# MariMamgo/CNN-with-PDE

Measured on AMD Instinct MI355X. Metric: PDE-layer fwd+bwd Msamples/s, higher is better.
Workload: dtype f32; 1 GPU; cifar10.EnhancedDiffusionLayer(size=32, channels=64, num_steps=10) fwd+bwd, 30 implicit sweeps, batch 512/GPU, channel mixing disabled (BASELINE configs[1], SURVEY §8d cfg2 primary); global_batch=512, parallelism=dp1, grad_allreduce_bytes=0, rccl_world_size=1

## Files before the change

cnn-with-pde_amd/csrc/blob_to_inc.py:

```python
#!/usr/bin/env python3
import sys

if "--fwd" in sys.argv:
    sys.argv.remove("--fwd")
    with open(sys.argv[1], "w") as out:
        rows = []
        for spec in sys.argv[2:]:
            name, path = spec.split("=", 1)
            data = open(path, "rb").read()
            out.write(f"alignas(4096) static const unsigned char kAsmFwdBlob_{name}[{len(data)}] = {{\n")
            for i in range(0, len(data), 32):
                out.write(",".join(str(b) for b in data[i:i + 32]) + ",\n")
            out.write("};\n")
            rows.append(f'    {{"{name}", {int(name.rstrip("t"))}, kAsmFwdBlob_{name}, "adi_fwd_asm_n32_w{name}", {{}}, {{}}}},')
        out.write("static Variant g_fwd_variants[] = {\n" + "\n".join(rows) + "\n};\n")
    sys.exit(0)

with open(sys.argv[1], "w") as out:
    rows = []
    for spec in sys.argv[2:]:
        name, path = spec.split("=", 1)
        data = open(path, "rb").read()
        nw = int(name.split("a")[0].rstrip("b"))
        out.write(f"alignas(4096) static const unsigned char kAsmBlob_{name}[{len(data)}] = {{\n")
        for i in range(0, len(data), 32):
            out.write(",".join(str(b) for b in data[i:i + 32]) + ",\n")
        out.write("};\n")
        rows.append(f'    {{"{name}", {nw}, kAsmBlob_{name}, "adi_bwd_asm_n32_w{name}", {{}}, {{}}}},')
    out.write("static Variant g_variants[] = {\n" + "\n".join(rows) + "\n};\n")
```

cnn-with-pde_amd/csrc/gen_adi_bwd_asm.py:

```python
#!/usr/bin/env python3
import sys

N = 32
M = 16
LINE = 36
IMG_B = 32 * LINE * 4
REC_STRIDE = 5 * 32 * LINE + 32
BWD_OFF_B = (32 * LINE) * 4
REC_WIN = 3 * 32 * LINE + 32
PIECES = (REC_WIN * 4 + 1023) // 1024
RECP_B = PIECES * 1024
OFF_JN = 0
OFF_E = 32 * 4
OFF_INV = (32 * LINE + 32) * 4
OFF_KAP = (2 * 32 * LINE + 32) * 4
NSLOT = 6
RING_B = NSLOT * RECP_B
TAB_DTS = 96 * 4
TAB_FIRST = 2 * 96 * 4
PLANE_B = N * N * 4


class Emit:
    def __init__(self):
        self.out = []
        self.lgkm = []
        self.vm = []
        self.smem = False
        self.nvalu = 0
        self.vop2_only = False

    def raw(self, s, comment=None):
        self.out.append("\t" + s + (f"\t; {comment}" if comment else ""))

    def label(self, name):
        self.out.append(f"{name}:")

    def comment(self, s):
        self.out.append(f"\t; {s}")

    @staticmethod
    def _last_hit(queue, regs):
        for i in range(len(queue) - 1, -1, -1):
            if queue[i] & regs:
                return i
        return None

    def need(self, regs):
        regs = set(regs)
        i = self._last_hit(self.lgkm, regs)
        if i is not None:
            n = len(self.lgkm) - 1 - i
            if self.smem:
                n = 0
            n = min(n, 15)
            self.raw(f"s_waitcnt lgkmcnt({n})")
            self.lgkm = self.lgkm[len(self.lgkm) - n:] if n else []
            if n == 0:
                self.smem = False
        i = self._last_hit(self.vm, regs)
        if i is not None:
            n = min(len(self.vm) - 1 - i, 63)
            self.raw(f"s_waitcnt vmcnt({n})")
            self.vm = self.vm[len(self.vm) - n:] if n else []

    def drain(self, vm=True, lgkm=True):
        parts = []
        if vm:
            parts.append("vmcnt(0)")
            self.vm = []
        if lgkm:
            parts.append("lgkmcnt(0)")
            self.lgkm = []
            self.smem = False
        self.raw("s_waitcnt " + " ".join(parts))

    def assert_idle(self):
        assert not self.lgkm and not self.vm and not self.smem, (len(self.lgkm), len(self.vm), self.smem)

    def valu(self, text, dst=(), src=(), comment=None):
        if self.vop2_only and text.startswith("v_fma_f32 "):
            ops = [o.strip() for o in text[len("v_fma_f32 "):].split(",")]
            text = f"v_fmac_f32 {ops[0]}, {ops[1].lstrip('-')}, {ops[2]}"
        self.need(set(dst) | set(src))
        self.raw(text, comment)
        self.nvalu += 1

    def salu(self, text, comment=None):
        self.raw(text, comment)

    def ds_read(self, text, dst, addr):
        self.need(set(dst) | {addr})
        self.raw(text)
        self.lgkm.append(set(dst))

    def ds_write(self, text, data, addr):
        self.need(set(data) | {addr})
        self.raw(text)
        self.lgkm.append(set())

    def vm_load(self, text, dst, addr):
        self.need(set(dst) | {addr})
        self.raw(text)
        self.vm.append(set(dst))

    def vm_store(self, text, data, addr):
        self.need(set(data) | {addr})
        self.raw(text)
        self.vm.append(set())

    def s_load(self, text):
        self.raw(text)
        self.smem = True
        self.lgkm.append(set())


def v(n):
    return f"v{n}"


def vq(n):
    return f"v[{n}:{n + 3}]"


def vp(n):
    return f"v[{n}:{n + 1}]"


def gen(NW, ABL=0, MODE="A"):
    """MODE "A": <= 168 VGPRs (three waves per SIMD with 12-wave workgroups), coefficient rows streamed four values at a time,
    one re-layout image per wave.  MODE "B": 256 VGPRs (two waves per SIMD, 8-wave workgroups): the three coefficient rows of
    a sweep are HELD in registers — fetched for the NEXT sweep as the current sweep's pass frees them, kept across the twin x
    sweeps of neighbouring time steps —, two images per wave so that the re-layout writes ride inside the G passes, the next
    chunk's planes prefetched into 64 registers during the chunk's last time step, the time-weighted sums updated in the
    latency shadow of the next sweep's junction exchange."""
    assert NW in (8, 12, 16) and MODE in ("A", "B")
    BM = MODE == "B"
    NT = NW * 64
    PPI = 2 * NW
    NPI = (3 * PIECES + NW - 1) // NW
    NIMG = 2 if BM else 1
    WIMG_B = NIMG * IMG_B
    IMG0 = 0
    RING0 = NW * WIMG_B
    ADT = BM and bool(ABL & 65536)
    assert (NW - 1) * WIMG_B < 65536
    FLAGS = BM and not (ABL & 16384)
    CNT0 = RING0 + RING_B
    LDS_TOTAL = CNT0 + (16 if FLAGS else 0)
    assert LDS_TOTAL <= 163840, LDS_TOTAL
    assert (NW - 1) * WIMG_B < 65536
    e = Emit()
    e.vop2_only = bool(ABL & 64)
    name = f"adi_bwd_asm_n32_w{NW}" + ("b" if BM else "") + (f"a{ABL}" if ABL else "")

    NMARK = 16

    def mark(i):
        if not (ABL & 4096):
            return
        assert i < NMARK
        lab = f"L_mark_{mark.n}"
        mark.n += 1
        e.drain(vm=False)
        e.salu(f"s_or_b32 s{S_T0}, s2, s3")
        e.salu(f"s_or_b32 s{S_T0}, s{S_T0}, s4")
        e.salu(f"s_sub_u32 s{S_T1}, s{S_Q}, s{S_G}")
        e.salu(f"s_xor_b32 s{S_T1}, s{S_T1}, s{S_g}")
        e.salu(f"s_or_b32 s{S_T0}, s{S_T0}, s{S_T1}")
        e.salu(f"s_xor_b32 s{S_T1}, s{S_KK}, 5")
        e.salu(f"s_or_b32 s{S_T0}, s{S_T0}, s{S_T1}")
        e.salu(f"s_cmp_lg_u32 s{S_T0}, 0")
        e.salu(f"s_cbranch_scc1 {lab}")
        e.raw(f"{'s_memrealtime' if ABL & 131072 else 's_memtime'} s[{S_STAMP}:{S_STAMP + 1}]")
        e.raw("s_waitcnt lgkmcnt(0)")
        a, b = NQ[0][0], NQ[0][1]
        e.raw(f"v_mov_b32 {v(a)}, s{S_STAMP}")
        e.raw(f"v_mov_b32 {v(b)}, s{S_STAMP + 1}")
        e.salu(f"s_mul_i32 s{S_T1}, s{S_WAVE}, {NMARK * 8}")
        e.salu(f"s_add_u32 s{S_T1}, s{S_T1}, {i * 8}")
        e.raw(f"v_mov_b32 {v(VADDR)}, s{S_T1}")
        assert NQ[0][1] == NQ[0][0] + 1 and NQ[0][0] % 2 == 0
        e.raw(f"global_store_dwordx2 {v(VADDR)}, v[{a}:{b}], s[{S_DBG}:{S_DBG + 1}]")
        e.raw("s_waitcnt vmcnt(0)")
        e.label(lab)
    mark.n = 0

    def stage(n):
        e.salu(f"s_cmp_eq_u32 s31, {n}")
        e.salu("s_cbranch_scc1 L_end")

    nv = [0]

    def alloc(n, align=1):
        nv[0] = (nv[0] + align - 1) // align * align
        r = nv[0]
        nv[0] += n
        return r

    R = [alloc(16, 4), alloc(16, 4)]
    X = [alloc(16, 4), alloc(16, 4)]
    AX, TX, AY, TY = alloc(16, 4), alloc(16, 4), alloc(16, 4), alloc(16, 4)
    if BM:
        CE, CI, CK = alloc(16, 4), alloc(16, 4), alloc(16, 4)
        EB = [CE, CE + 4]
        IB = [CI, CI + 4]
        KB = [CK, CK + 4]
    else:
        EB = [alloc(4, 4), alloc(4, 4)]
        IB = [alloc(4, 4), alloc(4, 4)]
        KB = [alloc(4, 4), alloc(4, 4)]
    _nq = alloc(4, 2)
    NQ = [[_nq, _nq + 1], [_nq + 2, _nq + 3]]
    JN = alloc(1)
    VADDR = alloc(1)
    if BM:
        VADDRN = alloc(1)
        VDTS = alloc(1)
    V_CROW = alloc(1)
    V_TWR = alloc(1)
    V_TRD = alloc(1)
    V_NKK, V_MU, V_MD = alloc(1), alloc(1), alloc(1)
    V_LANE16 = alloc(1)
    V_M2 = alloc(1)
    if BM:
        PF = alloc(64, 4)
        TQ = [CE + 4 * i for i in range(4)] + [CI + 4 * i for i in range(4)] + [CK + 4 * i for i in range(4)]
    else:
        TQ = [EB[0], EB[1], IB[0], IB[1], KB[0], KB[1]]
    NVGPR = nv[0]
    assert NVGPR <= (256 if BM else 168), NVGPR

    S_GY, S_Y, S_GU, S_COEF, S_PART, S_TAB, S_VAR = 8, 10, 12, 14, 16, 18, 20
    S_B, S_C, S_S, S_G, S_GUSC, S_ACCP, S_CZ, S_K, S_NCHUNK = 22, 23, 24, 25, 26, 27, 28, 29, 30
    S_c, S_g, S_WAVE, S_T, S_Q, S_KK, S_SET, S_MORE = 32, 33, 34, 35, 36, 37, 38, 39
    S_T0, S_T1, S_T2, S_T3 = 40, 41, 42, 43
    S_FIRSTX, S_FIRSTY, S_TLX, S_TLY = 44, 45, 46, 47
    S_SRC, S_SRC0 = 48, 50
    S_KKN = 52
    S_SWB, S_SWB3 = 53, 54
    S_DL = [56 + 2 * i for i in range(6)]
    S_DS = [57 + 2 * i for i in range(6)]
    S_PV = 68
    S_HASNEXT = 69
    S_PX = 55
    S_TSTEP = 5
    S_PB = [70, 72, 74, 76]
    S_VAL0, S_VAL1 = 78, 79
    S_DTS = [80, 81, 82]
    S_DTSB = 84
    S_REC = 86
    S_SS = 87
    S_A0 = 88
    S_IT = 90
    S_DBG = 92
    S_STAMP = 94
    NSGPR = 96

    e.out.append('\t.amdgcn_target "amdgcn-amd-amdhsa--gfx950"')
    e.out.append("\t.amdhsa_code_object_version 6")
    e.out.append("\t.text")
    e.out.append(f"\t.protected\t{name}")
    e.out.append(f"\t.globl\t{name}")
    e.out.append("\t.p2align\t8")
    e.out.append(f"\t.type\t{name},@function")
    e.label(name)

    e.s_load("s_load_dwordx16 s[8:23], s[0:1], 0x0")
    e.s_load("s_load_dwordx8 s[24:31], s[0:1], 0x40")
    if ABL & 4096:
        e.s_load(f"s_load_dwordx2 s[{S_DBG}:{S_DBG + 1}], s[0:1], 0x60")
    T0, T1, T2 = EB[0], EB[0] + 1, EB[0] + 2
    e.valu(f"v_bfe_u32 {v(T1)}, v0, 6, 4", dst=[T1])
    e.valu(f"v_and_b32 {v(T0)}, 63, v0", dst=[T0])
    e.raw("s_nop 1")
    e.valu(f"v_readfirstlane_b32 s{S_WAVE}, {v(T1)}", src=[T1])
    e.valu(f"v_lshlrev_b32 {v(V_LANE16)}, 4, {v(T0)}", dst=[V_LANE16], src=[T0])
    e.valu(f"v_and_b32 {v(T1)}, 31, {v(T0)}", dst=[T1], src=[T0])
    e.valu(f"v_lshrrev_b32 {v(T2)}, 5, {v(T0)}", dst=[T2], src=[T0])
    e.valu(f"v_mul_u32_u24 {v(V_CROW)}, 0x90, {v(T1)}", dst=[V_CROW], src=[T1])
    e.valu(f"v_lshl_add_u32 {v(V_CROW)}, {v(T2)}, 6, {v(V_CROW)}", dst=[V_CROW], src=[T2, V_CROW])
    T3 = EB[0] + 3
    e.valu(f"v_sub_u32 {v(T3)}, 47, {v(T1)}", dst=[T3], src=[T1])
    e.valu(f"v_cmp_gt_u32 vcc, 16, {v(T1)}", src=[T1])
    e.valu(f"v_cndmask_b32 {v(T3)}, {v(T3)}, {v(T1)}, vcc", dst=[T3], src=[T3, T1])
    e.salu(f"s_mul_i32 s{S_T}, s{S_WAVE}, {WIMG_B}")
    e.salu(f"s_add_u32 s{S_T}, s{S_T}, {IMG0}")
    e.valu(f"v_mul_u32_u24 {v(V_TWR)}, 0x900, {v(T2)}", dst=[V_TWR], src=[T2])
    e.valu(f"v_lshl_add_u32 {v(V_TWR)}, {v(T3)}, 2, {v(V_TWR)}", dst=[V_TWR], src=[T3, V_TWR])
    e.valu(f"v_add_u32 {v(V_TWR)}, s{S_T}, {v(V_TWR)}", dst=[V_TWR], src=[V_TWR])
    if ADT:
        TA, TB = IB[0], IB[0] + 1
        e.valu(f"v_sub_u32 {v(TA)}, 31, {v(T1)}", dst=[TA], src=[T1])
        e.valu(f"v_cmp_gt_u32 vcc, 16, {v(T1)}", src=[T1])
        e.valu(f"v_cndmask_b32 {v(TA)}, {v(TA)}, {v(T1)}, vcc", dst=[TA], src=[TA, T1])
        e.valu(f"v_cndmask_b32 {v(TB)}, 1, 0, vcc", dst=[TB])
        e.valu(f"v_add_u32 {v(V_TRD)}, 4, {v(TA)}", dst=[V_TRD], src=[TA])
        e.valu(f"v_lshrrev_b32 {v(V_TRD)}, 3, {v(V_TRD)}", dst=[V_TRD], src=[V_TRD])
        e.valu(f"v_lshl_add_u32 {v(V_TRD)}, {v(V_TRD)}, 3, {v(TA)}", dst=[V_TRD], src=[V_TRD, TA])
        e.valu(f"v_lshlrev_b32 {v(TA)}, 6, {v(TA)}", dst=[TA], src=[TA])
        e.valu(f"v_lshl_add_u32 {v(V_TRD)}, {v(V_TRD)}, 2, {v(TA)}", dst=[V_TRD], src=[V_TRD, TA])
        e.valu(f"v_lshl_add_u32 {v(V_TRD)}, {v(TB)}, 5, {v(V_TRD)}", dst=[V_TRD], src=[TB, V_TRD])
        e.valu(f"v_lshl_add_u32 {v(V_TRD)}, {v(T2)}, 4, {v(V_TRD)}", dst=[V_TRD], src=[T2, V_TRD])
        e.valu(f"v_lshlrev_b32 {v(V_TRD)}, 2, {v(V_TRD)}", dst=[V_TRD], src=[V_TRD])
        e.valu(f"v_add_u32 {v(V_TRD)}, s{S_T}, {v(V_TRD)}", dst=[V_TRD], src=[V_TRD])
    else:
        e.valu(f"v_mul_u32_u24 {v(V_TRD)}, 0x90, {v(T3)}", dst=[V_TRD], src=[T3])
        e.valu(f"v_lshl_add_u32 {v(V_TRD)}, {v(T2)}, 6, {v(V_TRD)}", dst=[V_TRD], src=[T2, V_TRD])
        e.valu(f"v_add_u32 {v(V_TRD)}, s{S_T}, {v(V_TRD)}", dst=[V_TRD], src=[V_TRD])
    e.valu(f"v_cmp_lt_u32 vcc, 0, {v(T1)}", src=[T1])
    e.valu(f"v_cndmask_b32 {v(V_MU)}, 0, 1.0, vcc", dst=[V_MU])
    e.valu(f"v_cmp_gt_u32 vcc, 31, {v(T1)}", src=[T1])
    e.valu(f"v_cndmask_b32 {v(V_MD)}, 0, 1.0, vcc", dst=[V_MD])
    e.valu(f"v_add_f32 {v(V_NKK)}, {v(V_MU)}, {v(V_MD)}", dst=[V_NKK], src=[V_MU, V_MD])
    e.valu(f"v_sub_f32 {v(V_NKK)}, 0, {v(V_NKK)}", dst=[V_NKK], src=[V_NKK])
    e.valu(f"v_mov_b32 {v(V_M2)}, -2.0", dst=[V_M2])
    for k in range(16):
        for a in (AX, TX, AY, TY):
            e.valu(f"v_mov_b32 {v(a + k)}, 0", dst=[a + k])
    for i in range(4):
        e.valu(f"v_mov_b32 {v(IB[0] + i)}, 0", dst=[IB[0] + i])
    e.valu(f"v_add_u32 {v(VADDR)}, s{S_T}, {v(V_LANE16)}", dst=[VADDR], src=[V_LANE16])
    for i in range(4):
        e.ds_write(f"ds_write_b128 {v(VADDR)}, {vq(IB[0])} offset:{1024 * i}", [IB[0] + j for j in range(4)], VADDR)
    e.valu(f"v_lshrrev_b32 {v(T0)}, 1, {v(V_LANE16)}", dst=[T0], src=[V_LANE16])
    e.valu(f"v_add_u32 {v(T0)}, s{S_T}, {v(T0)}", dst=[T0], src=[T0])
    e.ds_write(f"ds_write_b64 {v(T0)}, {vp(IB[0])} offset:4096", [IB[0], IB[0] + 1], T0)
    if BM:
        for i in range(4):
            e.ds_write(f"ds_write_b128 {v(VADDR)}, {vq(IB[0])} offset:{IMG_B + 1024 * i}", [IB[0] + j for j in range(4)], VADDR)
        e.ds_write(f"ds_write_b64 {v(T0)}, {vp(IB[0])} offset:{IMG_B + 4096}", [IB[0], IB[0] + 1], T0)
    e.drain(vm=False)
    stage(1)
    e.salu(f"s_mul_i32 s{S_T0}, s{S_CZ}, s4")
    e.salu(f"s_add_u32 s{S_c}, s2, s{S_T0}")
    e.salu(f"s_mov_b32 s{S_g}, s3")
    e.salu(f"s_lshl_b32 s{S_T0}, s{S_c}, 2")
    e.salu(f"s_add_u32 s{S_A0}, s{S_VAR}, s{S_T0}")
    e.salu(f"s_addc_u32 s{S_A0 + 1}, s{S_VAR + 1}, 0")
    e.s_load(f"s_load_dword s{S_T1}, s[{S_A0}:{S_A0 + 1}], 0x0")
    e.s_load(f"s_load_dwordx4 s[{S_FIRSTX}:{S_FIRSTX + 3}], s[{S_TAB}:{S_TAB + 1}], {hex(TAB_FIRST)}")
    e.drain(vm=False)
    e.salu(f"s_cmp_lg_u32 s{S_T1}, 0")
    e.salu("s_cbranch_scc1 L_end")
    stage(2)
    e.salu(f"s_add_u32 s{S_DTSB}, s{S_TAB}, {TAB_DTS}")
    e.salu(f"s_addc_u32 s{S_DTSB + 1}, s{S_TAB + 1}, 0")
    e.salu(f"s_mul_i32 s{S_SWB}, s{S_C}, {REC_STRIDE * 4}")
    e.salu(f"s_mul_i32 s{S_SWB3}, s{S_SWB}, 3")
    e.salu(f"s_mul_i32 s{S_T0}, s{S_c}, {REC_STRIDE * 4}")
    e.salu(f"s_mul_hi_u32 s{S_T1}, s{S_c}, {REC_STRIDE * 4}")
    e.salu(f"s_add_u32 s{S_T0}, s{S_T0}, {BWD_OFF_B}")
    e.salu(f"s_addc_u32 s{S_T1}, s{S_T1}, 0")
    e.salu(f"s_add_u32 s{S_SRC0}, s{S_COEF}, s{S_T0}")
    e.salu(f"s_addc_u32 s{S_SRC0 + 1}, s{S_COEF + 1}, s{S_T1}")
    e.salu(f"s_mov_b32 s{S_PV}, 0")
    e.salu(f"s_mov_b32 s{S_PX}, 0")
    for i in range(NPI):
        e.salu(f"s_add_u32 s{S_T0}, s{S_WAVE}, {NW * i}")
        e.salu(f"s_mul_i32 s{S_T1}, s{S_T0}, 4682")
        e.salu(f"s_lshr_b32 s{S_T1}, s{S_T1}, 16")
        e.salu(f"s_mul_i32 s{S_T2}, s{S_T1}, {PIECES}")
        e.salu(f"s_sub_u32 s{S_T2}, s{S_T0}, s{S_T2}")
        e.salu(f"s_lshl_b32 s{S_T2}, s{S_T2}, 10")
        e.salu(f"s_mul_i32 s{S_T3}, s{S_T1}, {RECP_B}")
        e.salu(f"s_add_u32 s{S_DL[i]}, s{S_T3}, s{S_T2}")
        e.salu(f"s_add_u32 s{S_DL[i]}, s{S_DL[i]}, {RING0}")
        e.salu(f"s_sub_u32 s{S_T3}, 2, s{S_T1}")
        e.salu(f"s_mul_i32 s{S_T3}, s{S_T3}, s{S_SWB}")
        e.salu(f"s_add_u32 s{S_DS[i]}, s{S_T3}, s{S_T2}")
        e.salu(f"s_cmp_lt_u32 s{S_T0}, {3 * PIECES}")
        e.salu(f"s_cselect_b32 s{S_T3}, {1 << i}, 0")
        e.salu(f"s_or_b32 s{S_PV}, s{S_PV}, s{S_T3}")
        e.salu(f"s_cmp_eq_u32 s{S_T1}, 0")
        e.salu(f"s_cselect_b32 s{S_T3}, {1 << i}, 0")
        e.salu(f"s_or_b32 s{S_PX}, s{S_PX}, s{S_T3}")

    def dma_step(kk_sgpr, set_expr_sgpr, skip_twin=False):
        e.salu(f"s_mul_i32 s{S_T0}, s{kk_sgpr}, s{S_SWB3}")
        e.salu(f"s_add_u32 s{S_SRC}, s{S_SRC0}, s{S_T0}")
        e.salu(f"s_addc_u32 s{S_SRC + 1}, s{S_SRC0 + 1}, 0")
        if skip_twin:
            e.salu(f"s_sub_u32 s{S_T0}, s{S_K}, 1")
            e.salu(f"s_cmp_eq_u32 s{kk_sgpr}, s{S_T0}")
            e.salu(f"s_cselect_b32 s{S_T1}, 0, s{S_PX}")
            e.salu(f"s_bitcmp1_b32 s{S_ACCP}, 1")
            e.salu(f"s_cselect_b32 s{S_T1}, s{S_T1}, 0")
            e.salu(f"s_andn2_b32 s{S_T3}, s{S_PV}, s{S_T1}")
        for i in range(NPI):
            last_partial = (NW * i + NW > 3 * PIECES)
            if skip_twin:
                e.salu(f"s_bitcmp1_b32 s{S_T3}, {i}")
                e.salu(f"s_cbranch_scc0 L_nodma_{dma_step.n}_{i}")
            elif last_partial:
                e.salu(f"s_bitcmp1_b32 s{S_PV}, {i}")
                e.salu(f"s_cbranch_scc0 L_nodma_{dma_step.n}_{i}")
            e.salu(f"s_add_u32 s{S_A0}, s{S_SRC}, s{S_DS[i]}")
            e.salu(f"s_addc_u32 s{S_A0 + 1}, s{S_SRC + 1}, 0")
            e.salu(f"s_add_u32 m0, s{set_expr_sgpr}, s{S_DL[i]}")
            e.salu("s_nop 0")
            e.raw(f"global_load_lds_dwordx4 {v(V_LANE16)}, s[{S_A0}:{S_A0 + 1}]")
            if last_partial or skip_twin:
                e.label(f"L_nodma_{dma_step.n}_{i}")
        dma_step.n += 1
    dma_step.n = 0

    def load_dts(kk_sgpr):
        e.salu(f"s_mul_i32 s{S_T0}, s{kk_sgpr}, 12")
        e.salu(f"s_add_u32 s{S_A0}, s{S_DTSB}, s{S_T0}")
        e.salu(f"s_addc_u32 s{S_A0 + 1}, s{S_DTSB + 1}, 0")
        e.s_load(f"s_load_dword s{S_DTS[0]}, s[{S_A0}:{S_A0 + 1}], 0x0")
        e.s_load(f"s_load_dword s{S_DTS[1]}, s[{S_A0}:{S_A0 + 1}], 0x4")
        e.s_load(f"s_load_dword s{S_DTS[2]}, s[{S_A0}:{S_A0 + 1}], 0x8")

    def flag_add(which, set_sgpr_is_other):
        a = VDTS
        e.salu(f"s_cmp_eq_u32 s{S_SET}, 0")
        e.salu(f"s_cselect_b32 s{S_T0}, {4 if set_sgpr_is_other else 0}, {0 if set_sgpr_is_other else 4}")
        e.salu(f"s_add_u32 s{S_T0}, s{S_T0}, {CNT0 + which * 8}")
        e.valu(f"v_mov_b32 {v(a)}, s{S_T0}", dst=[a])
        b = VADDR
        e.valu(f"v_mov_b32 {v(b)}, 1", dst=[b])
        e.need({a, b})
        e.raw("s_mov_b64 exec, 1")
        e.raw(f"ds_add_u32 {v(a)}, {v(b)}")
        e.raw("s_mov_b64 exec, -1")
        e.lgkm.append(set())

    def flag_wait(which, other_set, target_sgpr, tag):
        a, b = VDTS, VADDR
        e.drain(vm=False)
        e.salu(f"s_cmp_eq_u32 s{S_SET}, 0")
        e.salu(f"s_cselect_b32 s{S_T0}, {4 if other_set else 0}, {0 if other_set else 4}")
        e.salu(f"s_add_u32 s{S_T0}, s{S_T0}, {CNT0 + which * 8}")
        e.valu(f"v_mov_b32 {v(a)}, s{S_T0}", dst=[a])
        e.salu(f"s_mov_b32 s{S_T1}, 0")
        e.label(f"L_poll_{tag}")
        e.raw(f"ds_read_b32 {v(b)}, {v(a)}")
        e.raw("s_waitcnt lgkmcnt(0)")
        e.raw(f"v_readfirstlane_b32 s{S_T2}, {v(b)}")
        e.salu(f"s_cmp_ge_u32 s{S_T2}, s{target_sgpr}")
        e.salu(f"s_cbranch_scc1 L_polled_{tag}")
        e.salu(f"s_add_u32 s{S_T1}, s{S_T1}, 1")
        e.salu(f"s_cmp_lt_u32 s{S_T1}, 0x100000")
        e.salu(f"s_cbranch_scc0 L_polled_{tag}")
        e.raw("s_sleep 1")
        e.salu(f"s_branch L_poll_{tag}")
        e.label(f"L_polled_{tag}")

    if FLAGS:
        for i in range(4):
            e.valu(f"v_mov_b32 {v(IB[0] + i)}, 0", dst=[IB[0] + i])
        e.valu(f"v_mov_b32 {v(VADDR)}, {CNT0}", dst=[VADDR])
        e.ds_write(f"ds_write_b128 {v(VADDR)}, {vq(IB[0])}", [IB[0] + j for j in range(4)], VADDR)
        e.salu(f"s_mov_b32 s{S_TSTEP}, 0")
    if bool(ABL & 8192) != BM:
        e.salu(f"s_cmp_lt_u32 s{S_WAVE}, {NW // 2}")
        e.salu("s_cbranch_scc1 L_noprio")
        e.raw("s_setprio 1")
        e.label("L_noprio")
    stage(31)
    e.salu(f"s_mov_b32 s{S_SET}, 0")
    e.salu(f"s_sub_u32 s{S_KK}, s{S_K}, 1")
    dma_step(S_KK, S_SET)
    e.raw("s_waitcnt vmcnt(0)")
    stage(32)
    load_dts(S_KK)
    e.drain(vm=False)
    stage(33)
    e.salu(f"s_mov_b32 s{S_Q}, s{S_g}")
    e.drain()
    e.raw("s_barrier")
    if FLAGS:
        flag_add(0, False)
    stage(3)

    def plane_bases(ptr, dst_pairs, q_sgpr=None):
        q_sgpr = S_Q if q_sgpr is None else q_sgpr
        for j, d in enumerate(dst_pairs):
            e.salu(f"s_mul_i32 s{S_T0}, s{q_sgpr}, {PPI}")
            e.salu(f"s_lshl_b32 s{S_T1}, s{S_WAVE}, 1")
            e.salu(f"s_add_u32 s{S_T0}, s{S_T0}, s{S_T1}")
            if j:
                e.salu(f"s_add_u32 s{S_T0}, s{S_T0}, {j}")
            e.salu(f"s_sub_u32 s{S_T1}, s{S_B}, 1")
            e.salu(f"s_min_u32 s{S_T0}, s{S_T0}, s{S_T1}")
            e.salu(f"s_mul_i32 s{S_T0}, s{S_T0}, s{S_C}")
            e.salu(f"s_add_u32 s{S_T0}, s{S_T0}, s{S_c}")
            e.salu(f"s_lshr_b32 s{S_T1}, s{S_T0}, 20")
            e.salu(f"s_lshl_b32 s{S_T0}, s{S_T0}, 12")
            e.salu(f"s_add_u32 s{d}, s{ptr}, s{S_T0}")
            e.salu(f"s_addc_u32 s{d + 1}, s{ptr + 1}, s{S_T1}")

    def io_addresses():
        a, b = NQ[0][0], NQ[0][1]
        e.salu("s_mov_b32 vcc_lo, 0xf0f0f0f0")
        e.salu("s_mov_b32 vcc_hi, 0xf0f0f0f0")
        e.valu(f"v_lshrrev_b32 {v(a)}, 7, {v(V_LANE16)}", dst=[a], src=[V_LANE16])
        e.valu(f"v_mul_u32_u24 {v(a)}, 0x90, {v(a)}", dst=[a], src=[a])
        e.valu(f"v_and_b32 {v(b)}, 0x70, {v(V_LANE16)}", dst=[b], src=[V_LANE16])
        e.valu(f"v_sub_u32 {v(VADDR)}, 0xb0, {v(b)}", dst=[VADDR], src=[b])
        e.valu(f"v_cndmask_b32 {v(b)}, {v(b)}, {v(VADDR)}, vcc", dst=[b], src=[b, VADDR])
        e.valu(f"v_add3_u32 {v(VADDR)}, {v(a)}, {v(b)}, s{S_T}", dst=[VADDR], src=[a, b])
        e.valu(f"v_add_u32 {v(JN)}, s{S_T}, {v(V_CROW)}", dst=[JN], src=[V_CROW])

    def chunk_flags():
        e.salu(f"s_add_u32 s{S_T0}, s{S_Q}, s{S_G}")
        e.salu(f"s_cmp_lt_u32 s{S_T0}, s{S_NCHUNK}")
        e.salu(f"s_cselect_b32 s{S_MORE}, 1, 0")
        e.salu(f"s_mul_i32 s{S_T0}, s{S_Q}, {PPI}")
        e.salu(f"s_lshl_b32 s{S_T1}, s{S_WAVE}, 1")
        e.salu(f"s_add_u32 s{S_T0}, s{S_T0}, s{S_T1}")
        e.salu(f"s_cmp_lt_u32 s{S_T0}, s{S_B}")
        e.salu(f"s_cselect_b32 s{S_VAL0}, 1, 0")
        e.salu(f"s_add_u32 s{S_T0}, s{S_T0}, 1")
        e.salu(f"s_cmp_lt_u32 s{S_T0}, s{S_B}")
        e.salu(f"s_cselect_b32 s{S_VAL1}, 1, 0")

    def fetch_planes(regs, q_sgpr, tracked):
        plane_bases(S_GY, [S_PB[0], S_PB[1]], q_sgpr)
        plane_bases(S_Y, [S_PB[2], S_PB[3]], q_sgpr)
        for d, pb in zip(regs, S_PB):
            for i in range(4):
                text = f"global_load_dwordx4 {vq(d + 4 * i)}, {v(V_LANE16)}, s[{pb}:{pb + 1}] offset:{1024 * i} nt"
                if tracked:
                    e.vm_load(text, [d + 4 * i + j for j in range(4)], V_LANE16)
                else:
                    e.raw(text)

    def place_planes(regs):
        dests = [R[0], R[1], X[0], X[1]]
        io_addresses()
        for pi, (src, d) in enumerate(zip(regs, dests)):
            for i in range(4):
                t = TQ[(pi * 4 + i) % len(TQ)]
                a = src + 4 * i
                e.valu(f"v_cndmask_b32 {v(t)}, {v(a)}, {v(a + 3)}, vcc", dst=[t], src=[a, a + 3])
                e.valu(f"v_cndmask_b32 {v(t + 1)}, {v(a + 1)}, {v(a + 2)}, vcc", dst=[t + 1], src=[a + 1, a + 2])
                e.valu(f"v_cndmask_b32 {v(t + 2)}, {v(a + 2)}, {v(a + 1)}, vcc", dst=[t + 2], src=[a + 2, a + 1])
                e.valu(f"v_cndmask_b32 {v(t + 3)}, {v(a + 3)}, {v(a)}, vcc", dst=[t + 3], src=[a + 3, a])
                e.ds_write(f"ds_write_b128 {v(VADDR)}, {vq(t)} offset:{8 * LINE * 4 * i}", [t + j for j in range(4)], VADDR)
            for i in range(4):
                e.ds_read(f"ds_read_b128 {vq(d + 4 * i)}, {v(JN)} offset:{16 * i}", [d + 4 * i + j for j in range(4)], JN)
        e.drain(vm=False)
        for pj, sval in ((0, S_VAL0), (1, S_VAL1)):
            e.salu(f"s_cmp_eq_u32 s{sval}, 1")
            e.salu(f"s_cbranch_scc1 L_valid_{place_planes.n}_{pj}")
            for k in range(16):
                e.valu(f"v_mov_b32 {v(R[pj] + k)}, 0", dst=[R[pj] + k])
                e.valu(f"v_mov_b32 {v(X[pj] + k)}, 0", dst=[X[pj] + k])
            e.label(f"L_valid_{place_planes.n}_{pj}")
        place_planes.n += 1
    place_planes.n = 0

    def load_planes():
        e.comment("---- chunk in: gy -> R, y -> X (global -> natural image -> half rows)")
        chunk_flags()
        if BM:
            place_planes([PF, PF + 16, PF + 32, PF + 48])
        else:
            regs = [R[0], R[1], X[0], X[1]]
            fetch_planes(regs, S_Q, True)
            place_planes(regs)

    def store_planes():
        e.comment("---- chunk out: gu = R * (1+eps)^-S (half rows -> natural image -> global)")
        e.assert_idle()
        plane_bases(S_GU, [S_PB[0], S_PB[1]])
        io_addresses()
        for pj, sval in ((0, S_VAL0), (1, S_VAL1)):
            e.salu(f"s_cmp_eq_u32 s{sval}, 0")
            e.salu(f"s_cbranch_scc1 L_nostore_{store_planes.n}_{pj}")
            for k in range(16):
                e.valu(f"v_mul_f32 {v(R[pj] + k)}, s{S_GUSC}, {v(R[pj] + k)}", dst=[R[pj] + k], src=[R[pj] + k])
            for i in range(4):
                e.ds_write(f"ds_write_b128 {v(JN)}, {vq(R[pj] + 4 * i)} offset:{16 * i}", [R[pj] + 4 * i + j for j in range(4)], JN)
            for i in range(4):
                e.ds_read(f"ds_read_b128 {vq(X[pj] + 4 * i)}, {v(VADDR)} offset:{8 * LINE * 4 * i}",
                          [X[pj] + 4 * i + j for j in range(4)], VADDR)
            for i in range(4):
                a = X[pj] + 4 * i
                t = R[pj] + 4 * i
                e.valu(f"v_cndmask_b32 {v(t)}, {v(a)}, {v(a + 3)}, vcc", dst=[t], src=[a, a + 3])
                e.valu(f"v_cndmask_b32 {v(t + 1)}, {v(a + 1)}, {v(a + 2)}, vcc", dst=[t + 1], src=[a + 1, a + 2])
                e.valu(f"v_cndmask_b32 {v(t + 2)}, {v(a + 2)}, {v(a + 1)}, vcc", dst=[t + 2], src=[a + 2, a + 1])
                e.valu(f"v_cndmask_b32 {v(t + 3)}, {v(a + 3)}, {v(a)}, vcc", dst=[t + 3], src=[a + 3, a])
                e.raw(f"global_store_dwordx4 {v(V_LANE16)}, {vq(t)}, s[{S_PB[pj]}:{S_PB[pj] + 1}] offset:{1024 * i} nt")
            e.drain(vm=False)
            e.label(f"L_nostore_{store_planes.n}_{pj}")
        store_planes.n += 1
    store_planes.n = 0

    def q4(k):
        return k // 4

    def ebuf(k):
        return EB[q4(k) & 1] + (k & 3)

    def ibuf(k):
        return IB[q4(k) & 1] + (k & 3)

    def kbuf(k):
        return KB[q4(k) & 1] + (k & 3)

    def rd_quad(buf, off, q):
        if ABL & 2:
            return
        b = buf[q & 1]
        e.ds_read(f"ds_read_b128 {vq(b)}, {v(VADDR)} offset:{off + 16 * q}", [b + j for j in range(4)], VADDR)

    def sweep_addr(rec_index):
        e.salu(f"s_add_u32 s{S_REC}, s{S_SET}, {rec_index * RECP_B + RING0}")
        e.valu(f"v_add_u32 {v(VADDR)}, s{S_REC}, {v(V_CROW)}", dst=[VADDR], src=[V_CROW])
        t = NQ[0][0]
        e.valu(f"v_bfe_u32 {v(t)}, {v(V_LANE16)}, 2, 7", dst=[t], src=[V_LANE16])
        e.valu(f"v_add_u32 {v(t)}, s{S_REC}, {v(t)}", dst=[t], src=[t])
        if not (ABL & 2):
            e.ds_read(f"ds_read_b32 {v(JN)}, {v(t)} offset:{OFF_JN}", [JN], t)

    def xchg_pair(a, b):
        e.need({a, b})
        if ABL & 128:
            return
        if not (ABL & 32):
            e.raw("s_nop 1")
        e.raw(f"v_permlane32_swap_b32 {v(a)}, {v(b)}")
        if not (ABL & 32):
            e.raw("s_nop 1")
        e.raw(f"v_permlane32_swap_b32 {v(b)}, {v(a)}")
        if not (ABL & 32):
            e.raw("s_nop 1")
        e.nvalu += 2

    def h_pass(issue_hooks):
        for k in range(1, 16):
            for p in (0, 1):
                e.valu(f"v_fmac_f32 {v(R[p] + k)}, {v(ebuf(k - 1))}, {v(R[p] + k - 1)}",
                       dst=[R[p] + k], src=[R[p] + k, ebuf(k - 1), R[p] + k - 1])
            if k in issue_hooks:
                issue_hooks[k]()

    def junction():
        ta, tb = NQ[0][0], NQ[1][0]
        e.valu(f"v_mul_f32 {v(ta)}, {v(ebuf(15))}, {v(R[0] + 15)}", dst=[ta], src=[ebuf(15), R[0] + 15])
        e.valu(f"v_mul_f32 {v(tb)}, {v(ebuf(15))}, {v(R[1] + 15)}", dst=[tb], src=[ebuf(15), R[1] + 15])
        xchg_pair(ta, tb)
        e.valu(f"v_add_f32 {v(R[0] + 15)}, {v(R[0] + 15)}, {v(tb)}", dst=[R[0] + 15], src=[R[0] + 15, tb])
        e.valu(f"v_add_f32 {v(R[1] + 15)}, {v(R[1] + 15)}, {v(ta)}", dst=[R[1] + 15], src=[R[1] + 15, ta])
        e.valu(f"v_mul_f32 {v(R[0] + 15)}, {v(JN)}, {v(R[0] + 15)}", dst=[R[0] + 15], src=[JN, R[0] + 15])
        e.valu(f"v_mul_f32 {v(R[1] + 15)}, {v(JN)}, {v(R[1] + 15)}", dst=[R[1] + 15], src=[JN, R[1] + 15])

    def t_update(acc, tacc, dts_sgpr, first_sgpr, tlast_sgpr, tag):
        if ABL & 256:
            return
        lab = f"L_tu_{tag}_{t_update.n}"
        t_update.n += 1
        e.salu(f"s_cmp_eq_u32 s{S_SS}, s{first_sgpr}")
        e.salu(f"s_cselect_b32 s{S_T0}, s{S_MORE}, 0")
        e.salu(f"s_and_b32 s{S_T1}, s{dts_sgpr}, 0x7fffffff")
        e.salu(f"s_or_b32 s{S_T1}, s{S_T1}, s{S_T0}")
        e.salu(f"s_cmp_eq_u32 s{S_T1}, 0")
        e.salu(f"s_cbranch_scc1 {lab}_skip")
        e.valu(f"v_mov_b32 {v(JN)}, s{dts_sgpr}", dst=[JN])
        e.salu(f"s_cmp_eq_u32 s{S_T0}, 0")
        e.salu(f"s_cbranch_scc1 {lab}_noadj")
        e.valu(f"v_subrev_f32 {v(JN)}, s{tlast_sgpr}, {v(JN)}", dst=[JN], src=[JN])
        e.label(f"{lab}_noadj")
        for k in range(16):
            e.valu(f"v_fmac_f32 {v(tacc + k)}, {v(JN)}, {v(acc + k)}", dst=[tacc + k], src=[tacc + k, JN, acc + k])
        e.label(f"{lab}_skip")
    t_update.n = 0

    def sweep_x(rec_index, dts_sgpr):
        e.comment(f"==== x sweep, record {rec_index} of the set")
        sweep_addr(rec_index)
        rd_quad(EB, OFF_E, 0)
        rd_quad(EB, OFF_E, 1)
        rd_quad(IB, OFF_INV, 3)
        rd_quad(KB, OFF_KAP, 3)
        rd_quad(IB, OFF_INV, 2)
        rd_quad(KB, OFF_KAP, 2)
        e.valu(f"v_mov_b32 {v(NQ[0][1])}, {v(X[0] + 15)}", dst=[NQ[0][1]], src=[X[0] + 15])
        e.valu(f"v_mov_b32 {v(NQ[1][1])}, {v(X[1] + 15)}", dst=[NQ[1][1]], src=[X[1] + 15])
        xchg_pair(NQ[0][1], NQ[1][1])
        XIN = [NQ[1][1], NQ[0][1]]
        h_pass({4: lambda: rd_quad(EB, OFF_E, 2), 8: lambda: rd_quad(EB, OFF_E, 3)})
        junction()
        def nqreg(p, k):
            if k == 15:
                return XIN[p]
            return NQ[p][k & 1]
        pend = None
        for k in range(15, -1, -1):
            for p in (0, 1):
                nq = nqreg(p, k)
                if k == 15:
                    e.valu(f"v_add_f32 {v(nq)}, {v(nq)}, {v(X[p] + 14)}", dst=[nq], src=[nq, X[p] + 14])
                    e.valu(f"v_fmac_f32 {v(nq)}, {v(V_M2)}, {v(X[p] + 15)}", dst=[nq], src=[nq, V_M2, X[p] + 15])
                elif k == 0:
                    e.valu(f"v_sub_f32 {v(nq)}, {v(X[p] + 1)}, {v(X[p])}", dst=[nq], src=[X[p] + 1, X[p]])
                else:
                    e.valu(f"v_add_f32 {v(nq)}, {v(X[p] + k - 1)}, {v(X[p] + k + 1)}", dst=[nq], src=[X[p] + k - 1, X[p] + k + 1])
                    e.valu(f"v_fmac_f32 {v(nq)}, {v(V_M2)}, {v(X[p] + k)}", dst=[nq], src=[nq, V_M2, X[p] + k])
            if pend is not None:
                kk = pend
                for p in (0, 1):
                    e.valu(f"v_fma_f32 {v(X[p] + kk)}, -{v(kbuf(kk))}, {v(nqreg(p, kk))}, {v(X[p] + kk)}",
                           dst=[X[p] + kk], src=[kbuf(kk), nqreg(p, kk), X[p] + kk])
                if kk in (12, 8):
                    rd_quad(KB, OFF_KAP, q4(kk) - 2)
            if k >= 1:
                for p in (0, 1):
                    e.valu(f"v_fmac_f32 {v(R[p] + k - 1)}, {v(ebuf(k))}, {v(R[p] + k)}",
                           dst=[R[p] + k - 1], src=[R[p] + k - 1, ebuf(k), R[p] + k])
                if k in (12, 8):
                    rd_quad(EB, OFF_E, q4(k) - 2)
            for p in (0, 1):
                e.valu(f"v_mul_f32 {v(R[p] + k)}, {v(ibuf(k))}, {v(R[p] + k)}", dst=[R[p] + k], src=[ibuf(k), R[p] + k])
            if k in (12, 8):
                rd_quad(IB, OFF_INV, q4(k) - 2)
            for p in (0, 1):
                e.valu(f"v_fmac_f32 {v(AX + k)}, {v(R[p] + k)}, {v(nqreg(p, k))}", dst=[AX + k], src=[AX + k, R[p] + k, nqreg(p, k)])
            pend = k
        for p in (0, 1):
            e.valu(f"v_fma_f32 {v(X[p])}, -{v(kbuf(0))}, {v(nqreg(p, 0))}, {v(X[p])}", dst=[X[p]], src=[kbuf(0), nqreg(p, 0), X[p]])
        t_update(AX, TX, dts_sgpr, S_FIRSTX, S_TLX, "x")

    def relayout(arr):
        if ABL & 1:
            return
        for p in (0, 1):
            for k in range(16):
                e.ds_write(f"ds_write_b32 {v(V_TWR)}, {v(arr[p] + k)} offset:{k * LINE * 4}", [arr[p] + k], V_TWR)
            for i in range(4):
                e.ds_read(f"ds_read_b128 {vq(arr[p] + 4 * i)}, {v(V_TRD)} offset:{16 * i}", [arr[p] + 4 * i + j for j in range(4)], V_TRD)

    def sweep_y(rec_index, dts_sgpr):
        e.comment(f"==== y sweep, record {rec_index} of the set")
        sweep_addr(rec_index)
        rd_quad(EB, OFF_E, 0)
        rd_quad(EB, OFF_E, 1)
        rd_quad(IB, OFF_INV, 3)
        rd_quad(IB, OFF_INV, 2)
        relayout(R)
        h_pass({4: lambda: rd_quad(EB, OFF_E, 2), 8: lambda: rd_quad(EB, OFF_E, 3)})
        junction()
        for k in range(15, -1, -1):
            if k >= 1:
                for p in (0, 1):
                    e.valu(f"v_fmac_f32 {v(R[p] + k - 1)}, {v(ebuf(k))}, {v(R[p] + k)}",
                           dst=[R[p] + k - 1], src=[R[p] + k - 1, ebuf(k), R[p] + k])
                if k in (12, 8):
                    rd_quad(EB, OFF_E, q4(k) - 2)
            for p in (0, 1):
                e.valu(f"v_mul_f32 {v(R[p] + k)}, {v(ibuf(k))}, {v(R[p] + k)}", dst=[R[p] + k], src=[ibuf(k), R[p] + k])
            if k in (12, 8):
                rd_quad(IB, OFF_INV, q4(k) - 2)
        rd_quad(KB, OFF_KAP, 0)
        rd_quad(KB, OFF_KAP, 1)
        relayout(R)
        order = [(k, p) for k in range(16) for p in (0, 1)]
        GRP = 4
        for g0 in range(0, len(order), GRP):
            grp = order[g0:g0 + GRP]
            regs = [NQ[0][0], NQ[0][1], NQ[1][0], NQ[1][1]]
            for (k, p), nq in zip(grp, regs):
                e.valu(f"v_mul_f32 {v(nq)}, {v(V_NKK)}, {v(X[p] + k)}", dst=[nq], src=[V_NKK, X[p] + k])
            dpp_u = "" if ABL & 16 else " wave_shr:1 row_mask:0xf bank_mask:0xf bound_ctrl:0"
            dpp_d = "" if ABL & 16 else " wave_shl:1 row_mask:0xf bank_mask:0xf bound_ctrl:0"
            opc = "v_fmac_f32" if ABL & 16 else "v_fmac_f32_dpp"
            for (k, p), nq in zip(grp, regs):
                e.valu(f"{opc} {v(nq)}, {v(X[p] + k)}, {v(V_MU)}{dpp_u}", dst=[nq], src=[nq, X[p] + k, V_MU])
            for (k, p), nq in zip(grp, regs):
                e.valu(f"{opc} {v(nq)}, {v(X[p] + k)}, {v(V_MD)}{dpp_d}", dst=[nq], src=[nq, X[p] + k, V_MD])
            for (k, p), nq in zip(grp, regs):
                e.valu(f"v_fmac_f32 {v(AY + k)}, {v(R[p] + k)}, {v(nq)}", dst=[AY + k], src=[AY + k, R[p] + k, nq])
            for (k, p), nq in zip(grp, regs):
                e.valu(f"v_fma_f32 {v(X[p] + k)}, -{v(kbuf(k))}, {v(nq)}, {v(X[p] + k)}", dst=[X[p] + k], src=[kbuf(k), nq, X[p] + k])
            klast = grp[-1][0]
            if klast in (3, 7) and grp[-1][1] == 1:
                rd_quad(KB, OFF_KAP, q4(klast) + 2)
        t_update(AY, TY, dts_sgpr, S_FIRSTY, S_TLY, "y")

    def rd_row(base, off, q, addr):
        if ABL & 2:
            return
        e.ds_read(f"ds_read_b128 {vq(base + 4 * q)}, {v(addr)} offset:{off + 16 * q}", [base + 4 * q + j for j in range(4)], addr)

    def rec_addr(vreg, rec_index):
        e.salu(f"s_add_u32 s{S_REC}, s{S_SET}, {rec_index * RECP_B + RING0}")
        e.valu(f"v_add_u32 {v(vreg)}, s{S_REC}, {v(V_CROW)}", dst=[vreg], src=[V_CROW])

    def rd_jn(rec_index):
        if ABL & 2:
            return
        e.salu(f"s_add_u32 s{S_T0}, s{S_SET}, {rec_index * RECP_B + RING0}")
        e.valu(f"v_bfe_u32 {v(VDTS)}, {v(V_LANE16)}, 2, 7", dst=[VDTS], src=[V_LANE16])
        e.valu(f"v_add_u32 {v(VDTS)}, s{S_T0}, {v(VDTS)}", dst=[VDTS], src=[VDTS])
        e.ds_read(f"ds_read_b32 {v(JN)}, {v(VDTS)} offset:{OFF_JN}", [JN], VDTS)

    def load_rows_now(rec_index):
        rec_addr(VADDR, rec_index)
        rd_jn(rec_index)
        for q in range(4):
            rd_row(CE, OFF_E, q, VADDR)
        for q in range(4):
            rd_row(CI, OFF_INV, q, VADDR)
        for q in range(4):
            rd_row(CK, OFF_KAP, q, VADDR)

    def t_update_b(acc, tacc, dts_sgpr, first_sgpr, tlast_sgpr, ss_delta, tag):
        if ABL & 256:
            return
        lab = f"L_tub_{tag}_{t_update_b.n}"
        t_update_b.n += 1
        e.salu(f"s_add_u32 s{S_T2}, s{S_SS}, {ss_delta}")
        e.salu(f"s_cmp_eq_u32 s{S_T2}, s{first_sgpr}")
        e.salu(f"s_cselect_b32 s{S_T0}, s{S_MORE}, 0")
        e.salu(f"s_and_b32 s{S_T1}, s{dts_sgpr}, 0x7fffffff")
        e.salu(f"s_or_b32 s{S_T1}, s{S_T1}, s{S_T0}")
        e.salu(f"s_cmp_eq_u32 s{S_T1}, 0")
        e.salu(f"s_cbranch_scc1 {lab}_skip")
        e.valu(f"v_mov_b32 {v(VDTS)}, s{dts_sgpr}", dst=[VDTS])
        e.salu(f"s_cmp_eq_u32 s{S_T0}, 0")
        e.salu(f"s_cbranch_scc1 {lab}_noadj")
        e.valu(f"v_subrev_f32 {v(VDTS)}, s{tlast_sgpr}, {v(VDTS)}", dst=[VDTS], src=[VDTS])
        e.label(f"{lab}_noadj")
        for k in range(16):
            e.valu(f"v_fmac_f32 {v(tacc + k)}, {v(VDTS)}, {v(acc + k)}", dst=[tacc + k], src=[tacc + k, VDTS, acc + k])
        e.label(f"{lab}_skip")
    t_update_b.n = 0

    def swap(a, b):
        if ABL & 128:
            return
        e.need({a, b})
        e.raw(f"v_permlane32_swap_b32 {v(a)}, {v(b)}")
        e.nvalu += 1

    def nop2():
        if not (ABL & 32):
            e.raw("s_nop 1")

    def h_link(k):
        for p in (0, 1):
            e.valu(f"v_fmac_f32 {v(R[p] + k)}, {v(CE + k - 1)}, {v(R[p] + k - 1)}", dst=[R[p] + k], src=[R[p] + k, CE + k - 1, R[p] + k - 1])

    def junction_b(shadow1=None, shadow2=None, shadow3=None):
        ta, tb = NQ[0][0], NQ[1][0]
        e.valu(f"v_mul_f32 {v(ta)}, {v(CE + 15)}, {v(R[0] + 15)}", dst=[ta], src=[CE + 15, R[0] + 15])
        e.valu(f"v_mul_f32 {v(tb)}, {v(CE + 15)}, {v(R[1] + 15)}", dst=[tb], src=[CE + 15, R[1] + 15])
        if shadow1:
            shadow1()
        nop2()
        swap(ta, tb)
        if shadow2:
            shadow2()
        else:
            nop2()
        swap(tb, ta)
        if shadow3:
            shadow3()
        else:
            nop2()
        e.valu(f"v_add_f32 {v(R[0] + 15)}, {v(R[0] + 15)}, {v(tb)}", dst=[R[0] + 15], src=[R[0] + 15, tb])
        e.valu(f"v_add_f32 {v(R[1] + 15)}, {v(R[1] + 15)}, {v(ta)}", dst=[R[1] + 15], src=[R[1] + 15, ta])
        e.valu(f"v_mul_f32 {v(R[0] + 15)}, {v(JN)}, {v(R[0] + 15)}", dst=[R[0] + 15], src=[JN, R[0] + 15])
        e.valu(f"v_mul_f32 {v(R[1] + 15)}, {v(JN)}, {v(R[1] + 15)}", dst=[R[1] + 15], src=[JN, R[1] + 15])

    W2 = bool(ABL & 32768)

    ADT_P = [0, 1, 2, 3, 12, 13, 14, 15, 16, 17, 18, 19, 28, 29, 30, 31]

    def relayout_bases(upper):
        if ADT and not (ABL & 1):
            if upper:
                e.salu(f"s_mov_b32 m0, s{S_T}")
            return
        if not W2 or (ABL & 1):
            return
        if upper:
            e.valu(f"v_add_u32 {v(VDTS)}, {8 * LINE * 4}, {v(V_TWR)}", dst=[VDTS], src=[V_TWR])
            e.valu(f"v_add_u32 {v(VADDR)}, {8 * LINE * 4 + IMG_B}, {v(V_TWR)}", dst=[VADDR], src=[V_TWR])
        else:
            e.valu(f"v_add_u32 {v(VADDR)}, {IMG_B}, {v(V_TWR)}", dst=[VADDR], src=[V_TWR])

    def relayout_write(p, k):
        if ABL & 1:
            return
        if ADT:
            e.need({R[p] + k})
            e.raw(f"ds_write_addtid_b32 {v(R[p] + k)} offset:{4 * (64 * k + 4 * ADT_P[k]) + p * IMG_B}")
            e.lgkm.append(set())
            return
        if not W2:
            e.ds_write(f"ds_write_b32 {v(V_TWR)}, {v(R[p] + k)} offset:{k * LINE * 4 + p * IMG_B}", [R[p] + k], V_TWR)
            return
        if k & 1:
            return
        if k >= 8:
            base = VDTS if p == 0 else VADDR
        else:
            base = V_TWR if p == 0 else VADDR
        o0 = (k % 8) * LINE
        e.ds_write(f"ds_write2_b32 {v(base)}, {v(R[p] + k)}, {v(R[p] + k + 1)} offset0:{o0} offset1:{o0 + LINE}",
                   [R[p] + k, R[p] + k + 1], base)

    def relayout_reads():
        if ABL & 1:
            return
        for p in (0, 1):
            for i in range(4):
                e.ds_read(f"ds_read_b128 {vq(R[p] + 4 * i)}, {v(V_TRD)} offset:{16 * i + p * IMG_B}",
                          [R[p] + 4 * i + j for j in range(4)], V_TRD)

    def relayout_fix():
        if not ADT or (ABL & 1):
            return
        e.need(set(range(R[0], R[0] + 16)) | set(range(R[1], R[1] + 16)))
        e.raw("s_mov_b32 exec_lo, 0")
        for p in (0, 1):
            for j in range(8):
                e.raw(f"v_swap_b32 {v(R[p] + j)}, {v(R[p] + 15 - j)}")
                e.nvalu += 1
        e.raw("s_mov_b32 exec_lo, -1")

    def sweep_x_b(rec_index, next_rec, relayout_after, deferred, own_t):
        e.comment(f"==== x sweep (held rows), record {rec_index} of the set")
        if next_rec is not None:
            rec_addr(VADDRN, next_rec)
        e.valu(f"v_mov_b32 {v(NQ[0][1])}, {v(X[0] + 15)}", dst=[NQ[0][1]], src=[X[0] + 15])
        e.valu(f"v_mov_b32 {v(NQ[1][1])}, {v(X[1] + 15)}", dst=[NQ[1][1]], src=[X[1] + 15])
        h_link(1)
        swap(NQ[0][1], NQ[1][1])
        h_link(2)
        swap(NQ[1][1], NQ[0][1])
        XIN = [NQ[1][1], NQ[0][1]]
        for k in range(3, 16):
            h_link(k)

        def nqreg(p, k):
            return XIN[p] if k == 15 else NQ[p][k & 1]

        def nq15_a():
            for p in (0, 1):
                nq = nqreg(p, 15)
                e.valu(f"v_add_f32 {v(nq)}, {v(nq)}, {v(X[p] + 14)}", dst=[nq], src=[nq, X[p] + 14])

        def nq15_b():
            for p in (0, 1):
                nq = nqreg(p, 15)
                e.valu(f"v_fmac_f32 {v(nq)}, {v(V_M2)}, {v(X[p] + 15)}", dst=[nq], src=[nq, V_M2, X[p] + 15])

        sh1 = (lambda: t_update_b(*deferred)) if deferred else None
        junction_b(sh1, nq15_a, nq15_b)
        if next_rec is not None:
            rd_jn(next_rec)
        if relayout_after:
            relayout_bases(True)
        pend = None
        for k in range(15, -1, -1):
            if relayout_after and k == 7:
                relayout_bases(False)
            if k < 15:
                for p in (0, 1):
                    nq = nqreg(p, k)
                    if k == 0:
                        e.valu(f"v_sub_f32 {v(nq)}, {v(X[p] + 1)}, {v(X[p])}", dst=[nq], src=[X[p] + 1, X[p]])
                    else:
                        e.valu(f"v_add_f32 {v(nq)}, {v(X[p] + k - 1)}, {v(X[p] + k + 1)}", dst=[nq], src=[X[p] + k - 1, X[p] + k + 1])
                        e.valu(f"v_fmac_f32 {v(nq)}, {v(V_M2)}, {v(X[p] + k)}", dst=[nq], src=[nq, V_M2, X[p] + k])
            if pend is not None:
                kk_ = pend
                for p in (0, 1):
                    e.valu(f"v_fma_f32 {v(X[p] + kk_)}, -{v(CK + kk_)}, {v(nqreg(p, kk_))}, {v(X[p] + kk_)}",
                           dst=[X[p] + kk_], src=[CK + kk_, nqreg(p, kk_), X[p] + kk_])
                if next_rec is not None and kk_ % 4 == 0:
                    rd_row(CK, OFF_KAP, kk_ // 4, VADDRN)
            if k >= 1:
                for p in (0, 1):
                    e.valu(f"v_fmac_f32 {v(R[p] + k - 1)}, {v(CE + k)}, {v(R[p] + k)}", dst=[R[p] + k - 1], src=[R[p] + k - 1, CE + k, R[p] + k])
                if next_rec is not None:
                    if k % 4 == 0:
                        rd_row(CE, OFF_E, k // 4, VADDRN)
                    elif k == 1:
                        rd_row(CE, OFF_E, 0, VADDRN)
            for p in (0, 1):
                e.valu(f"v_mul_f32 {v(R[p] + k)}, {v(CI + k)}, {v(R[p] + k)}", dst=[R[p] + k], src=[CI + k, R[p] + k])
            if next_rec is not None and k % 4 == 0:
                rd_row(CI, OFF_INV, k // 4, VADDRN)
            if relayout_after:
                for p in (0, 1):
                    relayout_write(p, k)
            for p in (0, 1):
                e.valu(f"v_fmac_f32 {v(AX + k)}, {v(R[p] + k)}, {v(nqreg(p, k))}", dst=[AX + k], src=[AX + k, R[p] + k, nqreg(p, k)])
            pend = k
        if relayout_after:
            relayout_reads()
        for p in (0, 1):
            e.valu(f"v_fma_f32 {v(X[p])}, -{v(CK)}, {v(nqreg(p, 0))}, {v(X[p])}", dst=[X[p]], src=[CK, nqreg(p, 0), X[p]])
        if next_rec is not None:
            rd_row(CK, OFF_KAP, 0, VADDRN)
        if own_t:
            t_update_b(*own_t)
        if relayout_after:
            relayout_fix()

    def sweep_y_b(rec_index, next_rec, deferred):
        e.comment(f"==== y sweep (held rows), record {rec_index} of the set")
        rec_addr(VADDRN, next_rec)
        mark(7)
        for k in range(1, 16):
            h_link(k)
        mark(8)
        sh1 = (lambda: t_update_b(*deferred)) if deferred else None
        junction_b(sh1, None, None)
        rd_jn(next_rec)
        relayout_bases(True)
        for k in range(15, -1, -1):
            if k == 7:
                relayout_bases(False)
            if k >= 1:
                for p in (0, 1):
                    e.valu(f"v_fmac_f32 {v(R[p] + k - 1)}, {v(CE + k)}, {v(R[p] + k)}", dst=[R[p] + k - 1], src=[R[p] + k - 1, CE + k, R[p] + k])
                if k % 4 == 0:
                    rd_row(CE, OFF_E, k // 4, VADDRN)
                elif k == 1:
                    rd_row(CE, OFF_E, 0, VADDRN)
            for p in (0, 1):
                e.valu(f"v_mul_f32 {v(R[p] + k)}, {v(CI + k)}, {v(R[p] + k)}", dst=[R[p] + k], src=[CI + k, R[p] + k])
            if k % 4 == 0:
                rd_row(CI, OFF_INV, k // 4, VADDRN)
            for p in (0, 1):
                relayout_write(p, k)
        mark(9)
        relayout_reads()
        relayout_fix()
        mark(10)
        order = [(k, p) for k in range(16) for p in (0, 1)]
        GRP = 4
        dpp_u = "" if ABL & 16 else " wave_shr:1 row_mask:0xf bank_mask:0xf bound_ctrl:0"
        dpp_d = "" if ABL & 16 else " wave_shl:1 row_mask:0xf bank_mask:0xf bound_ctrl:0"
        opc = "v_fmac_f32" if ABL & 16 else "v_fmac_f32_dpp"
        regs = [NQ[0][0], NQ[0][1], NQ[1][0], NQ[1][1]]
        for g0 in range(0, len(order), GRP):
            grp = order[g0:g0 + GRP]
            for (k, p), nq in zip(grp, regs):
                e.valu(f"v_mul_f32 {v(nq)}, {v(V_NKK)}, {v(X[p] + k)}", dst=[nq], src=[V_NKK, X[p] + k])
            for (k, p), nq in zip(grp, regs):
                e.valu(f"{opc} {v(nq)}, {v(X[p] + k)}, {v(V_MU)}{dpp_u}", dst=[nq], src=[nq, X[p] + k, V_MU])
            for (k, p), nq in zip(grp, regs):
                e.valu(f"{opc} {v(nq)}, {v(X[p] + k)}, {v(V_MD)}{dpp_d}", dst=[nq], src=[nq, X[p] + k, V_MD])
            for (k, p), nq in zip(grp, regs):
                e.valu(f"v_fmac_f32 {v(AY + k)}, {v(R[p] + k)}, {v(nq)}", dst=[AY + k], src=[AY + k, R[p] + k, nq])
            for (k, p), nq in zip(grp, regs):
                e.valu(f"v_fma_f32 {v(X[p] + k)}, -{v(CK + k)}, {v(nq)}, {v(X[p] + k)}", dst=[X[p] + k], src=[CK + k, nq, X[p] + k])
            klast, plast = grp[-1]
            if plast == 1 and klast % 4 == 3:
                rd_row(CK, OFF_KAP, klast // 4, VADDRN)

    e.salu(f"s_cmp_lt_u32 s{S_Q}, s{S_NCHUNK}")
    e.salu("s_cbranch_scc0 L_epilogue")
    PFR = [PF, PF + 16, PF + 32, PF + 48] if BM else None
    if BM:
        fetch_planes(PFR, S_Q, False)
        e.raw("s_waitcnt vmcnt(0)")
    if ABL & 8:
        load_planes()
    e.label("L_chunk")
    if ABL & 8:
        e.salu(f"s_add_u32 s{S_T0}, s{S_Q}, s{S_G}")
        e.salu(f"s_cmp_lt_u32 s{S_T0}, s{S_NCHUNK}")
        e.salu(f"s_cselect_b32 s{S_MORE}, 1, 0")
    else:
        load_planes()
    stage(4)
    e.salu(f"s_sub_u32 s{S_KK}, s{S_K}, 1")
    e.label("L_step")
    e.assert_idle()
    mark(0)
    if FLAGS:
        e.salu(f"s_lshr_b32 s{S_T3}, s{S_TSTEP}, 1")
        e.salu(f"s_add_u32 s{S_T3}, s{S_T3}, 1")
        e.salu(f"s_mul_i32 s{S_T3}, s{S_T3}, {NW}")
        flag_wait(0, False, S_T3, "ready")
        e.salu(f"s_cmp_eq_u32 s{S_TSTEP}, 0")
        e.salu("s_cbranch_scc1 L_nodonewait")
        e.salu(f"s_sub_u32 s{S_T3}, s{S_TSTEP}, 1")
        e.salu(f"s_lshr_b32 s{S_T3}, s{S_T3}, 1")
        e.salu(f"s_add_u32 s{S_T3}, s{S_T3}, 1")
        e.salu(f"s_mul_i32 s{S_T3}, s{S_T3}, {NW}")
        flag_wait(1, True, S_T3, "done")
        e.label("L_nodonewait")
    e.salu(f"s_sub_u32 s{S_T0}, s{S_KK}, 1")
    e.salu(f"s_sub_u32 s{S_T1}, s{S_K}, 1")
    e.salu(f"s_cmp_gt_i32 s{S_KK}, 0")
    e.salu(f"s_cselect_b32 s{S_HASNEXT}, 1, s{S_MORE}")
    e.salu(f"s_cselect_b32 s{S_KKN}, s{S_T0}, s{S_T1}")
    if FLAGS:
        load_dts(S_KK)
    e.salu(f"s_cmp_eq_u32 s{S_HASNEXT}, 0")
    e.salu("s_cbranch_scc1 L_nonext")
    if not (ABL & 4) and not (ABL & 2048):
        e.salu(f"s_xor_b32 s{S_T2}, s{S_SET}, {3 * RECP_B}")
        dma_step(S_KKN, S_T2, skip_twin=BM)
    e.label("L_nonext")
    def prefetch_block():
        e.salu(f"s_cmp_eq_u32 s{S_KK}, 0")
        e.salu(f"s_cselect_b32 s{S_T0}, s{S_MORE}, 0")
        e.salu(f"s_cmp_eq_u32 s{S_T0}, 0")
        e.salu("s_cbranch_scc1 L_noprefetch")
        e.salu(f"s_add_u32 s{S_IT}, s{S_Q}, s{S_G}")
        fetch_planes(PFR, S_IT, False)
        e.label("L_noprefetch")

    if FLAGS:
        e.drain(vm=False)
    if BM and not (ABL & 8) and not FLAGS:
        e.salu(f"s_cmp_eq_u32 s{S_KK}, 0")
        e.salu(f"s_cselect_b32 s{S_T0}, s{S_MORE}, 0")
        e.salu(f"s_cmp_eq_u32 s{S_T0}, 0")
        e.salu("s_cbranch_scc1 L_noprefetch")
        e.salu(f"s_add_u32 s{S_IT}, s{S_Q}, s{S_G}")
        fetch_planes(PFR, S_IT, False)
        e.label("L_noprefetch")
    mark(1)
    e.salu(f"s_mul_i32 s{S_SS}, s{S_KK}, 3")
    e.salu(f"s_add_u32 s{S_SS}, s{S_SS}, 2")
    if BM:
        e.salu(f"s_sub_u32 s{S_T0}, s{S_K}, 1")
        e.salu(f"s_cmp_eq_u32 s{S_KK}, s{S_T0}")
        e.salu("s_cbranch_scc1 L_rows_now")
        e.salu(f"s_bitcmp1_b32 s{S_ACCP}, 1")
        e.salu("s_cbranch_scc1 L_rows_held")
        e.label("L_rows_now")
        load_rows_now(0)
        e.label("L_rows_held")
        sweep_x_b(0, 1, True, None, None)
        if FLAGS:
            e.raw("s_waitcnt vmcnt(0)")
            e.salu(f"s_cmp_eq_u32 s{S_HASNEXT}, 0")
            e.salu("s_cbranch_scc1 L_noready")
            flag_add(0, True)
            e.label("L_noready")
            if not (ABL & 8):
                prefetch_block()
        mark(2)
        e.salu(f"s_sub_u32 s{S_SS}, s{S_SS}, 1")
        sweep_y_b(1, 2, (AX, TX, S_DTS[2], S_FIRSTX, S_TLX, 1, "x2"))
        if FLAGS:
            flag_add(1, False)
        mark(3)
        e.salu(f"s_sub_u32 s{S_SS}, s{S_SS}, 1")
        sweep_x_b(2, None, False, (AY, TY, S_DTS[1], S_FIRSTY, S_TLY, 1, "y"), (AX, TX, S_DTS[0], S_FIRSTX, S_TLX, 0, "x0"))
        mark(4)
    else:
        sweep_x(0, S_DTS[2])
        mark(2)
        e.salu(f"s_sub_u32 s{S_SS}, s{S_SS}, 1")
        sweep_y(1, S_DTS[1])
        mark(3)
        e.salu(f"s_sub_u32 s{S_SS}, s{S_SS}, 1")
        sweep_x(2, S_DTS[0])
        mark(4)
    e.drain(vm=False)
    if FLAGS:
        e.salu(f"s_add_u32 s{S_TSTEP}, s{S_TSTEP}, 1")
        mark(5)
        mark(6)
    else:
        e.salu(f"s_cmp_eq_u32 s{S_HASNEXT}, 0")
        e.salu("s_cbranch_scc1 L_nodts")
        load_dts(S_KKN)
        e.label("L_nodts")
        e.raw("s_waitcnt vmcnt(0)")
        e.vm = []
        mark(5)
        if not (ABL & 4) and not (ABL & 1024):
            e.raw("s_barrier")
        e.drain(vm=False)
        mark(6)
    stage(5)
    if not (ABL & 4):
        e.salu(f"s_xor_b32 s{S_SET}, s{S_SET}, {3 * RECP_B}")
    e.salu(f"s_sub_u32 s{S_KK}, s{S_KK}, 1")
    e.salu(f"s_cmp_ge_i32 s{S_KK}, 0")
    e.salu("s_cbranch_scc1 L_step")
    stage(6)
    if FLAGS:
        e.raw("s_waitcnt vmcnt(0)")
    if not (ABL & 8):
        store_planes()
    stage(7)
    e.salu(f"s_add_u32 s{S_Q}, s{S_Q}, s{S_G}")
    e.salu(f"s_cmp_lt_u32 s{S_Q}, s{S_NCHUNK}")
    e.salu("s_cbranch_scc1 L_chunk")

    stage(8)
    e.label("L_epilogue")
    e.comment("---- epilogue: part[g][c][arr][image] = -(sum over waves), fixed order")
    e.drain()
    e.raw("s_barrier")
    e.salu(f"s_mul_i32 s{S_T0}, s{S_g}, s{S_C}")
    e.salu(f"s_add_u32 s{S_T0}, s{S_T0}, s{S_c}")
    e.salu(f"s_mul_hi_u32 s{S_T1}, s{S_T0}, {4 * IMG_B}")
    e.salu(f"s_mul_i32 s{S_T0}, s{S_T0}, {4 * IMG_B}")
    e.salu(f"s_add_u32 s{S_PB[0]}, s{S_PART}, s{S_T0}")
    e.salu(f"s_addc_u32 s{S_PB[0] + 1}, s{S_PART + 1}, s{S_T1}")
    VT4 = X[0]
    VSUM = X[0] + 1
    VOLD = X[0] + 2
    VA = X[0] + 3
    e.valu(f"v_lshrrev_b32 {v(VT4)}, 2, {v(V_LANE16)}", dst=[VT4], src=[V_LANE16])
    e.salu(f"s_lshl_b32 s{S_T0}, s{S_WAVE}, 8")
    e.valu(f"v_add_u32 {v(VT4)}, s{S_T0}, {v(VT4)}", dst=[VT4], src=[VT4])
    e.valu(f"v_add_u32 {v(JN)}, s{S_T}, {v(V_CROW)}", dst=[JN], src=[V_CROW])
    nit = (IMG_B // 4 + NT - 1) // NT
    for arr_i, arr in enumerate((AX, TX, AY, TY)):
        for i in range(4):
            e.ds_write(f"ds_write_b128 {v(JN)}, {vq(arr + 4 * i)} offset:{16 * i}", [arr + 4 * i + j for j in range(4)], JN)
        e.drain(vm=False)
        e.raw("s_barrier")
        for it in range(nit):
            first = it * NT
            nvalid = min(NT, IMG_B // 4 - first)
            lab = f"L_red_{arr_i}_{it}"
            if nvalid < NT:
                assert nvalid % 64 == 0
                e.salu(f"s_cmp_ge_u32 s{S_WAVE}, {nvalid // 64}")
                e.salu(f"s_cbranch_scc1 {lab}")
            e.valu(f"v_add_u32 {v(VA)}, {IMG0 + first * 4}, {v(VT4)}", dst=[VA], src=[VT4])
            tmp = [R[0] + w for w in range(NW)]
            for w in range(NW):
                e.ds_read(f"ds_read_b32 {v(tmp[w])}, {v(VA)} offset:{w * WIMG_B}", [tmp[w]], VA)
            e.valu(f"v_mov_b32 {v(VSUM)}, {v(tmp[0])}", dst=[VSUM], src=[tmp[0]])
            for w in range(1, NW):
                e.valu(f"v_add_f32 {v(VSUM)}, {v(VSUM)}, {v(tmp[w])}", dst=[VSUM], src=[VSUM, tmp[w]])
            e.valu(f"v_sub_f32 {v(VSUM)}, 0, {v(VSUM)}", dst=[VSUM], src=[VSUM])
            goff = arr_i * IMG_B + first * 4
            e.salu(f"s_add_u32 s{S_A0}, s{S_PB[0]}, {goff}")
            e.salu(f"s_addc_u32 s{S_A0 + 1}, s{S_PB[0] + 1}, 0")
            e.salu(f"s_bitcmp0_b32 s{S_ACCP}, 0")
            e.salu(f"s_cbranch_scc1 {lab}_noacc")
            e.vm_load(f"global_load_dword {v(VOLD)}, {v(VT4)}, s[{S_A0}:{S_A0 + 1}]", [VOLD], VT4)
            e.valu(f"v_add_f32 {v(VSUM)}, {v(VOLD)}, {v(VSUM)}", dst=[VSUM], src=[VOLD, VSUM])
            e.label(f"{lab}_noacc")
            e.raw(f"global_store_dword {v(VT4)}, {v(VSUM)}, s[{S_A0}:{S_A0 + 1}]")
            if nvalid < NT:
                e.label(lab)
        e.drain()
        e.raw("s_barrier")
    e.label("L_end")
    e.raw("s_endpgm")
    e.out.append("\t.p2alignl 6, 3212836864")
    e.out.append("\t.fill 256, 4, 3212836864")

    nvg = (NVGPR + 7) // 8 * 8
    desc = f"""
	.section	.rodata,"a",@progbits
	.p2align	6, 0x0
	.amdhsa_kernel {name}
		.amdhsa_group_segment_fixed_size {LDS_TOTAL}
		.amdhsa_private_segment_fixed_size 0
		.amdhsa_kernarg_size 104
		.amdhsa_user_sgpr_count 2
		.amdhsa_user_sgpr_dispatch_ptr 0
		.amdhsa_user_sgpr_queue_ptr 0
		.amdhsa_user_sgpr_kernarg_segment_ptr 1
		.amdhsa_user_sgpr_dispatch_id 0
		.amdhsa_user_sgpr_kernarg_preload_length 0
		.amdhsa_user_sgpr_kernarg_preload_offset 0
		.amdhsa_user_sgpr_private_segment_size 0
		.amdhsa_uses_dynamic_stack 0
		.amdhsa_enable_private_segment 0
		.amdhsa_system_sgpr_workgroup_id_x 1
		.amdhsa_system_sgpr_workgroup_id_y 1
		.amdhsa_system_sgpr_workgroup_id_z 1
		.amdhsa_system_sgpr_workgroup_info 0
		.amdhsa_system_vgpr_workitem_id 0
		.amdhsa_next_free_vgpr {nvg}
		.amdhsa_next_free_sgpr {NSGPR}
		.amdhsa_accum_offset {nvg}
		.amdhsa_reserve_vcc 1
		.amdhsa_float_round_mode_32 0
		.amdhsa_float_round_mode_16_64 0
		.amdhsa_float_denorm_mode_32 3
		.amdhsa_float_denorm_mode_16_64 3
		.amdhsa_dx10_clamp 1
		.amdhsa_ieee_mode 1
		.amdhsa_fp16_overflow 0
		.amdhsa_tg_split 0
		.amdhsa_exception_fp_ieee_invalid_op 0
		.amdhsa_exception_fp_denorm_src 0
		.amdhsa_exception_fp_ieee_div_zero 0
		.amdhsa_exception_fp_ieee_overflow 0
		.amdhsa_exception_fp_ieee_underflow 0
		.amdhsa_exception_fp_ieee_inexact 0
		.amdhsa_exception_int_div_zero 0
	.end_amdhsa_kernel
	.text
.Lfunc_end_{name}:
	.size	{name}, .Lfunc_end_{name}-{name}
	.amdgpu_metadata
---
amdhsa.kernels:
  - .agpr_count:     0
    .args:
      - .offset:         0
        .size:           104
        .value_kind:     by_value
    .group_segment_fixed_size: {LDS_TOTAL}
    .kernarg_segment_align: 8
    .kernarg_segment_size: 104
    .max_flat_workgroup_size: {NT}
    .name:           {name}
    .private_segment_fixed_size: 0
    .sgpr_count:     {NSGPR + 6}
    .sgpr_spill_count: 0
    .symbol:         {name}.kd
    .uniform_work_group_size: 1
    .uses_dynamic_stack: false
    .vgpr_count:     {nvg}
    .vgpr_spill_count: 0
    .wavefront_size: 64
amdhsa.target:   amdgcn-amd-amdhsa--gfx950
amdhsa.version:
  - 1
  - 2
...

	.end_amdgpu_metadata
"""
    info = dict(name=name, nvgpr=NVGPR, nvgpr_alloc=nvg, lds=LDS_TOTAL, nvalu=e.nvalu, nt=NT, ppi=PPI)
    return "\n".join(e.out) + "\n" + desc, info


if __name__ == "__main__":
    spec = sys.argv[1]
    head, _, abl = spec.partition("a")
    mode = "B" if head.endswith("b") else "A"
    text, info = gen(int(head.rstrip("b")), int(abl or 0), mode)
    with open(sys.argv[2], "w") as f:
        f.write(text)
    print(info, file=sys.stderr)
```

cnn-with-pde_amd/csrc/pde_adi_asm.hip:

```cpp
#include "pde_adi_asm.h"
#include "pde_common.h"

#include <cstdlib>
#include <mutex>
#include <string>

namespace pde {
namespace {

struct Variant {
    const char* spec;
    int nw;
    const unsigned char* blob;
    const char* name;
    hipModule_t mod[64];
    hipFunction_t fn[64];
};
#include "adi_bwd_asm_blob.inc"
#include "adi_fwd_asm_blob.inc"

Variant* chosen_fwd() {
    static Variant* v = [] () -> Variant* {
        const char* on = getenv("PDE_ASM_FWD");
        if (!on || on[0] != '1') return nullptr;
        const char* want = getenv("PDE_ASM_FWD_VARIANT");
        if (!want) return &g_fwd_variants[0];
        for (Variant& x : g_fwd_variants)
            if (std::string(want) == x.spec) return &x;
        return nullptr;
    }();
    return v;
}

Variant* chosen() {
    static Variant* v = [] () -> Variant* {
        const char* on = getenv("PDE_ASM_BWD");
        if (on && on[0] == '0') return nullptr;
        const char* want = getenv("PDE_ASM_VARIANT");
        std::string w = want ? want : "8b";
        for (Variant& x : g_variants)
            if (w == x.spec) return &x;
        return nullptr;
    }();
    return v;
}

hipFunction_t get_function(Variant& v) {
    static std::mutex mu;
    int dev = 0;
    if (hipGetDevice(&dev) != hipSuccess || dev < 0 || dev >= 64) return nullptr;
    std::lock_guard<std::mutex> lk(mu);
    if (!v.fn[dev]) {
        hipModule_t m = nullptr;
        hipFunction_t f = nullptr;
        if (hipModuleLoadData(&m, v.blob) != hipSuccess || hipModuleGetFunction(&f, m, v.name) != hipSuccess) {
            (void)hipGetLastError();
            return nullptr;
        }
        v.mod[dev] = m;
        v.fn[dev] = f;
    }
    return v.fn[dev];
}

void* stamp_buffer() {
    static void* buf = [] () -> void* {
        if (!getenv("PDE_ASM_STAMPS")) return nullptr;
        void* p = nullptr;
        if (hipMalloc(&p, 4096) != hipSuccess) return nullptr;
        (void)hipMemset(p, 0, 4096);
        return p;
    }();
    return buf;
}

}

extern "C" int pde_asm_stamps(unsigned long long* out, int n) {
    void* b = stamp_buffer();
    if (!b || n > 512) return -1;
    return hipMemcpy(out, b, (size_t)n * 8, hipMemcpyDeviceToHost) == hipSuccess ? 0 : -1;
}

int asm_bwd_waves() {
    Variant* v = chosen();
    return v ? v->nw : 0;
}

int asm_bwd_launch(int nw, const AsmBwdArgs& a, int xcd_map, hipStream_t st) {
    Variant* v = chosen();
    hipFunction_t fn = (v && v->nw == nw) ? get_function(*v) : nullptr;
    if (!fn) return PDE_E_LAUNCH;
    AsmBwdArgs args = a;
    args.cz_mul = xcd_map ? 8 : 0;
    static const int stop_stage = [] { const char* e = getenv("PDE_ASM_STAGE"); return e ? atoi(e) : 0; }();
    args.pad = stop_stage;
    args.dbg = stamp_buffer();
    size_t size = sizeof(args);
    void* extra[] = {HIP_LAUNCH_PARAM_BUFFER_POINTER, &args, HIP_LAUNCH_PARAM_BUFFER_SIZE, &size, HIP_LAUNCH_PARAM_END};
    const unsigned gx = xcd_map ? 8u : (unsigned)a.C, gz = xcd_map ? (unsigned)(a.C / 8) : 1u;
    if (hipModuleLaunchKernel(fn, gx, (unsigned)a.G, gz, (unsigned)(nw * 64), 1, 1, 0, st, nullptr, extra) != hipSuccess) {
        (void)hipGetLastError();
        return PDE_E_LAUNCH;
    }
    return PDE_OK;
}

bool asm_fwd_enabled() { return chosen_fwd() != nullptr; }

int asm_fwd_launch(const AsmBwdArgs& a, int xcd_map, hipStream_t st) {
    Variant* v = chosen_fwd();
    hipFunction_t fn = v ? get_function(*v) : nullptr;
    if (!fn) return PDE_E_LAUNCH;
    const unsigned threads = (unsigned)v->nw * 64u;
    AsmBwdArgs args = a;
    args.cz_mul = xcd_map ? 8 : 0;
    static const int stop_stage = [] { const char* e = getenv("PDE_ASM_FWD_STAGE"); return e ? atoi(e) : 0; }();
    args.pad = stop_stage;
    args.dbg = nullptr;
    size_t size = sizeof(args);
    void* extra[] = {HIP_LAUNCH_PARAM_BUFFER_POINTER, &args, HIP_LAUNCH_PARAM_BUFFER_SIZE, &size, HIP_LAUNCH_PARAM_END};
    const unsigned gx = xcd_map ? 8u : (unsigned)a.C, gz = xcd_map ? (unsigned)(a.C / 8) : 1u;
    if (hipModuleLaunchKernel(fn, gx, (unsigned)a.G, gz, threads, 1, 1, 0, st, nullptr, extra) != hipSuccess) {
        (void)hipGetLastError();
        return PDE_E_LAUNCH;
    }
    return PDE_OK;
}

}
```

Before: 1.131 Msamples/s.

## Add MODE C backward ADI asm kernel with scalar work hoisted out of time step

```diff
diff --git a/cnn-with-pde_amd/csrc/blob_to_inc.py b/cnn-with-pde_amd/csrc/blob_to_inc.py
--- a/cnn-with-pde_amd/csrc/blob_to_inc.py
+++ b/cnn-with-pde_amd/csrc/blob_to_inc.py
@@ -21,7 +21,7 @@
     for spec in sys.argv[2:]:
         name, path = spec.split("=", 1)
         data = open(path, "rb").read()
-        nw = int(name.split("a")[0].rstrip("b"))
+        nw = int(name.split("a")[0].rstrip("bc"))
         out.write(f"alignas(4096) static const unsigned char kAsmBlob_{name}[{len(data)}] = {{\n")
         for i in range(0, len(data), 32):
             out.write(",".join(str(b) for b in data[i:i + 32]) + ",\n")
diff --git a/cnn-with-pde_amd/csrc/gen_adi_bwd_asm.py b/cnn-with-pde_amd/csrc/gen_adi_bwd_asm.py
--- a/cnn-with-pde_amd/csrc/gen_adi_bwd_asm.py
+++ b/cnn-with-pde_amd/csrc/gen_adi_bwd_asm.py
@@ -22,6 +22,8 @@
 
 
 class Emit:
+    HAZ = 2
+
     def __init__(self):
         self.out = []
         self.lgkm = []
@@ -29,12 +31,45 @@
         self.smem = False
         self.nvalu = 0
         self.vop2_only = False
-
-    def raw(self, s, comment=None):
+        self.hist = []
+        self.pending = {}
+        self.count_haz = False
+
+    def _slot(self, writes=frozenset(), swap=False):
+        self.hist.append((frozenset(writes), swap))
+        del self.hist[:-self.HAZ]
+
+    def raw(self, s, comment=None, writes=frozenset(), swap=False):
         self.out.append("\t" + s + (f"\t; {comment}" if comment else ""))
+        op = s.split()[0]
+        if op == "s_nop":
+            for _ in range(int(s.split()[1]) + 1):
+                self._slot()
+            return
+        self._slot(writes, swap)
+        if op.startswith("s_cbranch") or op == "s_branch":
+            self.pending.setdefault(s.split()[1], []).append(list(self.hist))
 
     def label(self, name):
         self.out.append(f"{name}:")
+        for h in self.pending.pop(name, []):
+            a, b = [None] * (self.HAZ - len(self.hist)) + self.hist, [None] * (self.HAZ - len(h)) + h
+            self.hist = [(x or (frozenset(), False)) if y is None else (y if x is None else (x[0] | y[0], x[1] or y[1]))
+                         for x, y in zip(a, b)]
+
+    def wait_states(self, reads, swap):
+        reads = set(reads)
+        for d, (w, was_swap) in enumerate(reversed(self.hist)):
+            if w & reads and (swap or was_swap):
+                self.raw(f"s_nop {self.HAZ - d - 1}")
+                return
+
+    def ool(self, fn):
+        out, hist = self.out, list(self.hist)
+        self.out = []
+        fn()
+        text, self.out, self.hist = self.out, out, hist
+        return text
 
     def comment(self, s):
         self.out.append(f"\t; {s}")
@@ -83,7 +118,9 @@
             ops = [o.strip() for o in text[len("v_fma_f32 "):].split(",")]
             text = f"v_fmac_f32 {ops[0]}, {ops[1].lstrip('-')}, {ops[2]}"
         self.need(set(dst) | set(src))
-        self.raw(text, comment)
+        if self.count_haz:
+            self.wait_states(src, False)
+        self.raw(text, comment, writes=dst)
         self.nvalu += 1
 
     def salu(self, text, comment=None):
@@ -133,9 +170,13 @@
     a sweep are HELD in registers — fetched for the NEXT sweep as the current sweep's pass frees them, kept across the twin x
     sweeps of neighbouring time steps —, two images per wave so that the re-layout writes ride inside the G passes, the next
     chunk's planes prefetched into 64 registers during the chunk's last time step, the time-weighted sums updated in the
-    latency shadow of the next sweep's junction exchange."""
-    assert NW in (8, 12, 16) and MODE in ("A", "B")
-    BM = MODE == "B"
+    latency shadow of the next sweep's junction exchange.  MODE "C": MODE B's arithmetic in the same order per element, with
+    the scalar work taken out of the time step (bases per chunk, running record / table pointers, the counter targets
+    carried from step to step, one poll for both counters, the rare paths out of line) and the wait states of the lane
+    exchanges counted by `Emit` instead of fixed `s_nop`s."""
+    assert NW in (8, 12, 16) and MODE in ("A", "B", "C")
+    BM = MODE in ("B", "C")
+    SC = MODE == "C"
     NT = NW * 64
     PPI = 2 * NW
     NPI = (3 * PIECES + NW - 1) // NW
@@ -152,7 +193,9 @@
     assert (NW - 1) * WIMG_B < 65536
     e = Emit()
     e.vop2_only = bool(ABL & 64)
-    name = f"adi_bwd_asm_n32_w{NW}" + ("b" if BM else "") + (f"a{ABL}" if ABL else "")
+    e.count_haz = SC
+    name = f"adi_bwd_asm_n32_w{NW}" + {"A": "", "B": "b", "C": "c"}[MODE] + (f"a{ABL}" if ABL else "")
+    assert not (SC and ABL & (4 | 8 | 2048 | 8192 | 16384 | 65536)), "diagnostic bits of MODE B only"
 
     NMARK = 16
 
@@ -187,6 +230,8 @@
     mark.n = 0
 
     def stage(n):
+        if SC:
+            return
         e.salu(f"s_cmp_eq_u32 s31, {n}")
         e.salu("s_cbranch_scc1 L_end")
 
@@ -256,6 +301,15 @@
     S_DBG = 92
     S_STAMP = 94
     NSGPR = 96
+    if SC:
+        S_CNTC, S_CNTO = 6, 7
+        S_RT, S_DT = S_TSTEP, S_KKN
+        S_AJ = [96, 97, 98]
+        S_PVH = 99
+        S_SRCTOP = 100
+        S_RNKK = 31
+        S_PFKK = 91
+        NSGPR = 102
 
     e.out.append('\t.amdgcn_target "amdgcn-amd-amdhsa--gfx950"')
     e.out.append("\t.amdhsa_code_object_version 6")
@@ -375,6 +429,12 @@
         e.salu(f"s_cmp_eq_u32 s{S_T1}, 0")
         e.salu(f"s_cselect_b32 s{S_T3}, {1 << i}, 0")
         e.salu(f"s_or_b32 s{S_PX}, s{S_PX}, s{S_T3}")
+    if SC:
+        e.salu(f"s_sub_u32 s{S_T1}, s{S_K}, 1")
+        e.salu(f"s_bitcmp1_b32 s{S_ACCP}, 1")
+        e.salu(f"s_cselect_b32 s{S_T0}, s{S_PX}, 0")
+        e.salu(f"s_cselect_b32 s{S_RNKK}, s{S_T1}, 0")
+        e.salu(f"s_andn2_b32 s{S_PVH}, s{S_PV}, s{S_T0}")
 
     def dma_step(kk_sgpr, set_expr_sgpr, skip_twin=False):
         e.salu(f"s_mul_i32 s{S_T0}, s{kk_sgpr}, s{S_SWB3}")
@@ -405,6 +465,20 @@
         dma_step.n += 1
     dma_step.n = 0
 
+    def dma_step_sc(set_sgpr, mask_sgpr):
+        for i in range(NPI):
+            maybe = NW * i < PIECES or NW * i + NW > 3 * PIECES
+            if maybe:
+                e.salu(f"s_bitcmp1_b32 s{mask_sgpr}, {i}")
+                e.salu(f"s_cbranch_scc0 L_nodma_{dma_step.n}_{i}")
+            e.salu(f"s_add_u32 m0, s{set_sgpr}, s{S_DL[i]}")
+            e.salu(f"s_add_u32 s{S_A0}, s{S_SRC}, s{S_DS[i]}")
+            e.salu(f"s_addc_u32 s{S_A0 + 1}, s{S_SRC + 1}, 0")
+            e.raw(f"global_load_lds_dwordx4 {v(V_LANE16)}, s[{S_A0}:{S_A0 + 1}]")
+            if maybe:
+                e.label(f"L_nodma_{dma_step.n}_{i}")
+        dma_step.n += 1
+
     def load_dts(kk_sgpr):
         e.salu(f"s_mul_i32 s{S_T0}, s{kk_sgpr}, 12")
         e.salu(f"s_add_u32 s{S_A0}, s{S_DTSB}, s{S_T0}")
@@ -448,12 +522,53 @@
         e.salu(f"s_branch L_poll_{tag}")
         e.label(f"L_polled_{tag}")
 
+    def flag_add_sc(addr_sgpr, off):
+        e.valu(f"v_mov_b32 {v(VDTS)}, s{addr_sgpr}", dst=[VDTS])
+        e.valu(f"v_mov_b32 {v(VADDR)}, 1", dst=[VADDR])
+        e.need({VDTS, VADDR})
+        e.raw("s_mov_b64 exec, 1")
+        e.raw(f"ds_add_u32 {v(VDTS)}, {v(VADDR)}" + (f" offset:{off}" if off else ""))
+        e.raw("s_mov_b64 exec, -1")
+        e.lgkm.append(set())
+
+    def flag_poll_sc():
+        a, b = NQ[0][0], NQ[0][1]
+        e.assert_idle()
+        e.valu(f"v_mov_b32 {v(VDTS)}, s{S_CNTC}", dst=[VDTS])
+        e.salu(f"s_mov_b32 s{S_T1}, 0")
+        e.label("L_poll")
+        e.raw(f"ds_read2_b32 {vp(a)}, {v(VDTS)} offset1:2")
+        e.raw("s_waitcnt lgkmcnt(0)")
+        e.raw(f"v_readfirstlane_b32 s{S_T2}, {v(a)}")
+        e.raw(f"v_readfirstlane_b32 s{S_T3}, {v(b)}")
+        e.salu(f"s_cmp_lt_u32 s{S_T2}, s{S_RT}")
+        e.salu("s_cbranch_scc1 L_poll_wait")
+        e.salu(f"s_cmp_lt_u32 s{S_T3}, s{S_DT}")
+        e.salu("s_cbranch_scc1 L_poll_wait")
+        e.label("L_polled")
+
+        def tail():
+            e.label("L_poll_wait")
+            e.salu(f"s_add_u32 s{S_T1}, s{S_T1}, 1")
+            e.salu(f"s_cmp_lt_u32 s{S_T1}, 0x100000")
+            e.salu("s_cbranch_scc0 L_polled")
+            e.raw("s_sleep 1")
+            e.salu("s_branch L_poll")
+        OOL.append(e.ool(tail))
+
+    OOL = []
     if FLAGS:
         for i in range(4):
             e.valu(f"v_mov_b32 {v(IB[0] + i)}, 0", dst=[IB[0] + i])
         e.valu(f"v_mov_b32 {v(VADDR)}, {CNT0}", dst=[VADDR])
         e.ds_write(f"ds_write_b128 {v(VADDR)}, {vq(IB[0])}", [IB[0] + j for j in range(4)], VADDR)
-        e.salu(f"s_mov_b32 s{S_TSTEP}, 0")
+        if SC:
+            e.salu(f"s_mov_b32 s{S_CNTC}, {CNT0}")
+            e.salu(f"s_mov_b32 s{S_CNTO}, {CNT0 + 4}")
+            e.salu(f"s_mov_b32 s{S_RT}, {NW}")
+            e.salu(f"s_mov_b32 s{S_DT}, 0")
+        else:
+            e.salu(f"s_mov_b32 s{S_TSTEP}, 0")
     if bool(ABL & 8192) != BM:
         e.salu(f"s_cmp_lt_u32 s{S_WAVE}, {NW // 2}")
         e.salu("s_cbranch_scc1 L_noprio")
@@ -471,7 +586,10 @@
     e.salu(f"s_mov_b32 s{S_Q}, s{S_g}")
     e.drain()
     e.raw("s_barrier")
-    if FLAGS:
+    if SC:
+        e.salu(f"s_mov_b64 s[{S_SRCTOP}:{S_SRCTOP + 1}], s[{S_SRC}:{S_SRC + 1}]")
+        flag_add_sc(S_CNTC, 0)
+    elif FLAGS:
         flag_add(0, False)
     stage(3)
 
@@ -782,9 +900,10 @@
                 rd_quad(KB, OFF_KAP, q4(klast) + 2)
         t_update(AY, TY, dts_sgpr, S_FIRSTY, S_TLY, "y")
 
-    def rd_row(base, off, q, addr):
+    def rd_row(base, off, q, addr, rec=0):
         if ABL & 2:
             return
+        off += rec * RECP_B if SC else 0
         e.ds_read(f"ds_read_b128 {vq(base + 4 * q)}, {v(addr)} offset:{off + 16 * q}", [base + 4 * q + j for j in range(4)], addr)
 
     def rec_addr(vreg, rec_index):
@@ -799,7 +918,22 @@
         e.valu(f"v_add_u32 {v(VDTS)}, s{S_T0}, {v(VDTS)}", dst=[VDTS], src=[VDTS])
         e.ds_read(f"ds_read_b32 {v(JN)}, {v(VDTS)} offset:{OFF_JN}", [JN], VDTS)
 
+    def jn_addr():
+        e.valu(f"v_bfe_u32 {v(VDTS)}, {v(V_LANE16)}, 2, 7", dst=[VDTS], src=[V_LANE16])
+        e.valu(f"v_add_u32 {v(VDTS)}, s{S_REC}, {v(VDTS)}", dst=[VDTS], src=[VDTS])
+
+    def jn_load(rec_index):
+        if not (ABL & 2):
+            e.ds_read(f"ds_read_b32 {v(JN)}, {v(VDTS)} offset:{rec_index * RECP_B + OFF_JN}", [JN], VDTS)
+
     def load_rows_now(rec_index):
+        if SC:
+            jn_addr()
+            jn_load(rec_index)
+            for base, off in ((CE, OFF_E), (CI, OFF_INV), (CK, OFF_KAP)):
+                for q in range(4):
+                    rd_row(base, off, q, VADDRN, rec_index)
+            return
         rec_addr(VADDR, rec_index)
         rd_jn(rec_index)
         for q in range(4):
@@ -808,6 +942,28 @@
             rd_row(CI, OFF_INV, q, VADDR)
         for q in range(4):
             rd_row(CK, OFF_KAP, q, VADDR)
+
+    def t_update_sc(acc, tacc, dts_sgpr, aj_sgpr, tlast_sgpr, tag):
+        if ABL & 256:
+            return
+        lab = f"L_tuc_{tag}_{t_update_b.n}"
+        t_update_b.n += 1
+        e.salu(f"s_cmp_eq_u32 s{S_SS}, s{aj_sgpr}")
+        e.salu(f"s_cbranch_scc1 {lab}_adj")
+
+        def adj():
+            e.label(f"{lab}_adj")
+            e.valu(f"v_mov_b32 {v(VDTS)}, s{dts_sgpr}", dst=[VDTS])
+            e.valu(f"v_subrev_f32 {v(VDTS)}, s{tlast_sgpr}, {v(VDTS)}", dst=[VDTS], src=[VDTS])
+            e.salu(f"s_branch {lab}_fma")
+        OOL.append(e.ool(adj))
+        e.salu(f"s_lshl_b32 s{S_T1}, s{dts_sgpr}, 1")
+        e.salu(f"s_cbranch_scc0 {lab}_skip")
+        e.valu(f"v_mov_b32 {v(VDTS)}, s{dts_sgpr}", dst=[VDTS])
+        e.label(f"{lab}_fma")
+        for k in range(16):
+            e.valu(f"v_fmac_f32 {v(tacc + k)}, {v(VDTS)}, {v(acc + k)}", dst=[tacc + k], src=[tacc + k, VDTS, acc + k])
+        e.label(f"{lab}_skip")
 
     def t_update_b(acc, tacc, dts_sgpr, first_sgpr, tlast_sgpr, ss_delta, tag):
         if ABL & 256:
@@ -830,16 +986,19 @@
             e.valu(f"v_fmac_f32 {v(tacc + k)}, {v(VDTS)}, {v(acc + k)}", dst=[tacc + k], src=[tacc + k, VDTS, acc + k])
         e.label(f"{lab}_skip")
     t_update_b.n = 0
+    t_upd = t_update_sc if SC else t_update_b
 
     def swap(a, b):
         if ABL & 128:
             return
         e.need({a, b})
-        e.raw(f"v_permlane32_swap_b32 {v(a)}, {v(b)}")
+        if SC and not (ABL & 32):
+            e.wait_states({a, b}, True)
+        e.raw(f"v_permlane32_swap_b32 {v(a)}, {v(b)}", writes={a, b}, swap=True)
         e.nvalu += 1
 
     def nop2():
-        if not (ABL & 32):
+        if not (ABL & 32) and not SC:
             e.raw("s_nop 1")
 
     def h_link(k):
@@ -927,7 +1086,7 @@
 
     def sweep_x_b(rec_index, next_rec, relayout_after, deferred, own_t):
         e.comment(f"==== x sweep (held rows), record {rec_index} of the set")
-        if next_rec is not None:
+        if next_rec is not None and not SC:
             rec_addr(VADDRN, next_rec)
         e.valu(f"v_mov_b32 {v(NQ[0][1])}, {v(X[0] + 15)}", dst=[NQ[0][1]], src=[X[0] + 15])
         e.valu(f"v_mov_b32 {v(NQ[1][1])}, {v(X[1] + 15)}", dst=[NQ[1][1]], src=[X[1] + 15])
@@ -952,10 +1111,12 @@
                 nq = nqreg(p, 15)
                 e.valu(f"v_fmac_f32 {v(nq)}, {v(V_M2)}, {v(X[p] + 15)}", dst=[nq], src=[nq, V_M2, X[p] + 15])
 
-        sh1 = (lambda: t_update_b(*deferred)) if deferred else None
+        sh1 = (lambda: t_upd(*deferred)) if deferred else None
+        if SC and sh1 is None and next_rec is not None:
+            sh1 = jn_addr
         junction_b(sh1, nq15_a, nq15_b)
         if next_rec is not None:
-            rd_jn(next_rec)
+            jn_load(next_rec) if SC else rd_jn(next_rec)
         if relayout_after:
             relayout_bases(True)
         pend = None
@@ -976,19 +1137,19 @@
                     e.valu(f"v_fma_f32 {v(X[p] + kk_)}, -{v(CK + kk_)}, {v(nqreg(p, kk_))}, {v(X[p] + kk_)}",
                            dst=[X[p] + kk_], src=[CK + kk_, nqreg(p, kk_), X[p] + kk_])
                 if next_rec is not None and kk_ % 4 == 0:
-                    rd_row(CK, OFF_KAP, kk_ // 4, VADDRN)
+                    rd_row(CK, OFF_KAP, kk_ // 4, VADDRN, next_rec)
             if k >= 1:
                 for p in (0, 1):
                     e.valu(f"v_fmac_f32 {v(R[p] + k - 1)}, {v(CE + k)}, {v(R[p] + k)}", dst=[R[p] + k - 1], src=[R[p] + k - 1, CE + k, R[p] + k])
                 if next_rec is not None:
                     if k % 4 == 0:
-                        rd_row(CE, OFF_E, k // 4, VADDRN)
+                        rd_row(CE, OFF_E, k // 4, VADDRN, next_rec)
                     elif k == 1:
-                        rd_row(CE, OFF_E, 0, VADDRN)
+                        rd_row(CE, OFF_E, 0, VADDRN, next_rec)
             for p in (0, 1):
                 e.valu(f"v_mul_f32 {v(R[p] + k)}, {v(CI + k)}, {v(R[p] + k)}", dst=[R[p] + k], src=[CI + k, R[p] + k])
             if next_rec is not None and k % 4 == 0:
-                rd_row(CI, OFF_INV, k // 4, VADDRN)
+                rd_row(CI, OFF_INV, k // 4, VADDRN, next_rec)
             if relayout_after:
                 for p in (0, 1):
                     relayout_write(p, k)
@@ -1000,22 +1161,28 @@
         for p in (0, 1):
             e.valu(f"v_fma_f32 {v(X[p])}, -{v(CK)}, {v(nqreg(p, 0))}, {v(X[p])}", dst=[X[p]], src=[CK, nqreg(p, 0), X[p]])
         if next_rec is not None:
-            rd_row(CK, OFF_KAP, 0, VADDRN)
+            rd_row(CK, OFF_KAP, 0, VADDRN, next_rec)
         if own_t:
-            t_update_b(*own_t)
+            t_upd(*own_t)
         if relayout_after:
             relayout_fix()
 
     def sweep_y_b(rec_index, next_rec, deferred):
         e.comment(f"==== y sweep (held rows), record {rec_index} of the set")
-        rec_addr(VADDRN, next_rec)
+        if not SC:
+            rec_addr(VADDRN, next_rec)
         mark(7)
         for k in range(1, 16):
             h_link(k)
         mark(8)
-        sh1 = (lambda: t_update_b(*deferred)) if deferred else None
-        junction_b(sh1, None, None)
-        rd_jn(next_rec)
+        sh1 = (lambda: t_upd(*deferred)) if deferred else None
+        if SC:
+            junction_b(sh1, lambda: e.valu(f"v_bfe_u32 {v(VDTS)}, {v(V_LANE16)}, 2, 7", dst=[VDTS], src=[V_LANE16]),
+                       lambda: e.valu(f"v_add_u32 {v(VDTS)}, s{S_REC}, {v(VDTS)}", dst=[VDTS], src=[VDTS]))
+            jn_load(next_rec)
+        else:
+            junction_b(sh1, None, None)
+            rd_jn(next_rec)
         relayout_bases(True)
         for k in range(15, -1, -1):
             if k == 7:
@@ -1024,13 +1191,13 @@
                 for p in (0, 1):
                     e.valu(f"v_fmac_f32 {v(R[p] + k - 1)}, {v(CE + k)}, {v(R[p] + k)}", dst=[R[p] + k - 1], src=[R[p] + k - 1, CE + k, R[p] + k])
                 if k % 4 == 0:
-                    rd_row(CE, OFF_E, k // 4, VADDRN)
+                    rd_row(CE, OFF_E, k // 4, VADDRN, next_rec)
                 elif k == 1:
-                    rd_row(CE, OFF_E, 0, VADDRN)
+                    rd_row(CE, OFF_E, 0, VADDRN, next_rec)
             for p in (0, 1):
                 e.valu(f"v_mul_f32 {v(R[p] + k)}, {v(CI + k)}, {v(R[p] + k)}", dst=[R[p] + k], src=[CI + k, R[p] + k])
             if k % 4 == 0:
-                rd_row(CI, OFF_INV, k // 4, VADDRN)
+                rd_row(CI, OFF_INV, k // 4, VADDRN, next_rec)
             for p in (0, 1):
                 relayout_write(p, k)
         mark(9)
@@ -1057,7 +1224,73 @@
                 e.valu(f"v_fma_f32 {v(X[p] + k)}, -{v(CK + k)}, {v(nq)}, {v(X[p] + k)}", dst=[X[p] + k], src=[CK + k, nq, X[p] + k])
             klast, plast = grp[-1]
             if plast == 1 and klast % 4 == 3:
-                rd_row(CK, OFF_KAP, klast // 4, VADDRN)
+                rd_row(CK, OFF_KAP, klast // 4, VADDRN, next_rec)
+
+    def step_sc():
+        e.salu(f"s_mul_i32 s{S_SS}, s{S_KK}, 3")
+        flag_poll_sc()
+        e.salu(f"s_add_u32 s{S_REC}, s{S_SET}, {RING0}")
+        e.valu(f"v_add_u32 {v(VADDRN)}, s{S_REC}, {v(V_CROW)}", dst=[VADDRN], src=[V_CROW])
+        e.salu(f"s_sub_u32 s{S_SRC}, s{S_SRC}, s{S_SWB3}")
+        e.salu(f"s_subb_u32 s{S_SRC + 1}, s{S_SRC + 1}, 0")
+        e.salu(f"s_cmp_gt_i32 s{S_KK}, 0")
+        e.salu(f"s_cselect_b32 s{S_HASNEXT}, 1, s{S_MORE}")
+        e.salu(f"s_cselect_b64 s[{S_SRC}:{S_SRC + 1}], s[{S_SRC}:{S_SRC + 1}], s[{S_SRCTOP}:{S_SRCTOP + 1}]")
+        e.salu(f"s_cselect_b32 s{S_T3}, s{S_PVH}, s{S_PV}")
+        e.salu(f"s_mul_i32 s{S_T0}, s{S_KK}, 12")
+        e.s_load(f"s_load_dwordx4 s[{S_DTS[0]}:{S_DTS[0] + 3}], s[{S_DTSB}:{S_DTSB + 1}], s{S_T0}")
+        e.salu(f"s_cmp_eq_u32 s{S_HASNEXT}, 0")
+        e.salu("s_cbranch_scc1 L_nonext")
+        if not (ABL & 4) and not (ABL & 2048):
+            e.salu(f"s_xor_b32 s{S_T2}, s{S_SET}, {3 * RECP_B}")
+            dma_step_sc(S_T2, S_T3)
+        e.label("L_nonext")
+        e.drain(vm=False)
+        mark(1)
+        e.salu(f"s_cmp_ge_u32 s{S_KK}, s{S_RNKK}")
+        e.salu("s_cbranch_scc0 L_rows_held")
+        load_rows_now(0)
+        e.label("L_rows_held")
+        sweep_x_b(0, 1, True, None, None)
+        e.raw("s_waitcnt vmcnt(0)")
+        e.salu(f"s_cmp_eq_u32 s{S_HASNEXT}, 0")
+        e.salu("s_cbranch_scc1 L_noready")
+        flag_add_sc(S_CNTO, 0)
+        e.label("L_noready")
+        if not (ABL & 8):
+            e.salu(f"s_cmp_eq_u32 s{S_KK}, s{S_PFKK}")
+            e.salu("s_cbranch_scc1 L_prefetch")
+
+            def prefetch():
+                e.label("L_prefetch")
+                for d, pb in zip(PFR, S_PB):
+                    for i in range(4):
+                        e.raw(f"global_load_dwordx4 {vq(d + 4 * i)}, {v(V_LANE16)}, s[{pb}:{pb + 1}] offset:{1024 * i} nt")
+                e.salu("s_branch L_noprefetch")
+            OOL.append(e.ool(prefetch))
+            e.label("L_noprefetch")
+        mark(2)
+        sweep_y_b(1, 2, (AX, TX, S_DTS[2], S_AJ[0], S_TLX, "x2"))
+        flag_add_sc(S_CNTO, 8)
+        mark(3)
+        sweep_x_b(2, None, False, (AY, TY, S_DTS[1], S_AJ[1], S_TLY, "y"), (AX, TX, S_DTS[0], S_AJ[2], S_TLX, "x0"))
+        mark(4)
+        e.drain(vm=False)
+        e.salu(f"s_add_u32 s{S_T0}, s{S_DT}, {NW}")
+        e.salu(f"s_mov_b32 s{S_DT}, s{S_RT}")
+        e.salu(f"s_mov_b32 s{S_RT}, s{S_T0}")
+        e.salu(f"s_xor_b32 s{S_CNTC}, s{S_CNTC}, 4")
+        e.salu(f"s_xor_b32 s{S_CNTO}, s{S_CNTO}, 4")
+        mark(5)
+        mark(6)
+        e.salu(f"s_xor_b32 s{S_SET}, s{S_SET}, {3 * RECP_B}")
+        e.salu(f"s_sub_u32 s{S_KK}, s{S_KK}, 1")
+        e.salu(f"s_cmp_ge_i32 s{S_KK}, 0")
+        e.salu("s_cbranch_scc1 L_step")
+        e.salu("s_branch L_step_end")
+        for block in OOL:
+            e.out.extend(block)
+        e.label("L_step_end")
 
     e.salu(f"s_cmp_lt_u32 s{S_Q}, s{S_NCHUNK}")
     e.salu("s_cbranch_scc0 L_epilogue")
@@ -1075,117 +1308,131 @@
     else:
         load_planes()
     stage(4)
+    if SC:
+        e.salu(f"s_add_u32 s{S_IT}, s{S_Q}, s{S_G}")
+        plane_bases(S_GY, [S_PB[0], S_PB[1]], S_IT)
+        plane_bases(S_Y, [S_PB[2], S_PB[3]], S_IT)
+        e.salu(f"s_sub_u32 s{S_AJ[0]}, s{S_FIRSTX}, 2")
+        e.salu(f"s_sub_u32 s{S_AJ[1]}, s{S_FIRSTY}, 1")
+        e.salu(f"s_cmp_lg_u32 s{S_MORE}, 0")
+        e.salu(f"s_cselect_b32 s{S_AJ[0]}, s{S_AJ[0]}, -1")
+        e.salu(f"s_cselect_b32 s{S_AJ[1]}, s{S_AJ[1]}, -1")
+        e.salu(f"s_cselect_b32 s{S_AJ[2]}, s{S_FIRSTX}, -1")
+        e.salu(f"s_cselect_b32 s{S_PFKK}, 0, -1")
     e.salu(f"s_sub_u32 s{S_KK}, s{S_K}, 1")
     e.label("L_step")
     e.assert_idle()
     mark(0)
-    if FLAGS:
-        e.salu(f"s_lshr_b32 s{S_T3}, s{S_TSTEP}, 1")
-        e.salu(f"s_add_u32 s{S_T3}, s{S_T3}, 1")
-        e.salu(f"s_mul_i32 s{S_T3}, s{S_T3}, {NW}")
-        flag_wait(0, False, S_T3, "ready")
-        e.salu(f"s_cmp_eq_u32 s{S_TSTEP}, 0")
-        e.salu("s_cbranch_scc1 L_nodonewait")
-        e.salu(f"s_sub_u32 s{S_T3}, s{S_TSTEP}, 1")
-        e.salu(f"s_lshr_b32 s{S_T3}, s{S_T3}, 1")
-        e.salu(f"s_add_u32 s{S_T3}, s{S_T3}, 1")
-        e.salu(f"s_mul_i32 s{S_T3}, s{S_T3}, {NW}")
-        flag_wait(1, True, S_T3, "done")
-        e.label("L_nodonewait")
-    e.salu(f"s_sub_u32 s{S_T0}, s{S_KK}, 1")
-    e.salu(f"s_sub_u32 s{S_T1}, s{S_K}, 1")
-    e.salu(f"s_cmp_gt_i32 s{S_KK}, 0")
-    e.salu(f"s_cselect_b32 s{S_HASNEXT}, 1, s{S_MORE}")
-    e.salu(f"s_cselect_b32 s{S_KKN}, s{S_T0}, s{S_T1}")
-    if FLAGS:
-        load_dts(S_KK)
-    e.salu(f"s_cmp_eq_u32 s{S_HASNEXT}, 0")
-    e.salu("s_cbranch_scc1 L_nonext")
-    if not (ABL & 4) and not (ABL & 2048):
-        e.salu(f"s_xor_b32 s{S_T2}, s{S_SET}, {3 * RECP_B}")
-        dma_step(S_KKN, S_T2, skip_twin=BM)
-    e.label("L_nonext")
-    def prefetch_block():
-        e.salu(f"s_cmp_eq_u32 s{S_KK}, 0")
-        e.salu(f"s_cselect_b32 s{S_T0}, s{S_MORE}, 0")
-        e.salu(f"s_cmp_eq_u32 s{S_T0}, 0")
-        e.salu("s_cbranch_scc1 L_noprefetch")
-        e.salu(f"s_add_u32 s{S_IT}, s{S_Q}, s{S_G}")
-        fetch_planes(PFR, S_IT, False)
-        e.label("L_noprefetch")
-
-    if FLAGS:
+    if SC:
+        step_sc()
+    else:
+        if FLAGS:
+            e.salu(f"s_lshr_b32 s{S_T3}, s{S_TSTEP}, 1")
+            e.salu(f"s_add_u32 s{S_T3}, s{S_T3}, 1")
+            e.salu(f"s_mul_i32 s{S_T3}, s{S_T3}, {NW}")
+            flag_wait(0, False, S_T3, "ready")
+            e.salu(f"s_cmp_eq_u32 s{S_TSTEP}, 0")
+            e.salu("s_cbranch_scc1 L_nodonewait")
+            e.salu(f"s_sub_u32 s{S_T3}, s{S_TSTEP}, 1")
+            e.salu(f"s_lshr_b32 s{S_T3}, s{S_T3}, 1")
+            e.salu(f"s_add_u32 s{S_T3}, s{S_T3}, 1")
+            e.salu(f"s_mul_i32 s{S_T3}, s{S_T3}, {NW}")
+            flag_wait(1, True, S_T3, "done")
+            e.label("L_nodonewait")
+        e.salu(f"s_sub_u32 s{S_T0}, s{S_KK}, 1")
+        e.salu(f"s_sub_u32 s{S_T1}, s{S_K}, 1")
+        e.salu(f"s_cmp_gt_i32 s{S_KK}, 0")
+        e.salu(f"s_cselect_b32 s{S_HASNEXT}, 1, s{S_MORE}")
+        e.salu(f"s_cselect_b32 s{S_KKN}, s{S_T0}, s{S_T1}")
+        if FLAGS:
+            load_dts(S_KK)
+        e.salu(f"s_cmp_eq_u32 s{S_HASNEXT}, 0")
+        e.salu("s_cbranch_scc1 L_nonext")
+        if not (ABL & 4) and not (ABL & 2048):
+            e.salu(f"s_xor_b32 s{S_T2}, s{S_SET}, {3 * RECP_B}")
+            dma_step(S_KKN, S_T2, skip_twin=BM)
+        e.label("L_nonext")
+        def prefetch_block():
+            e.salu(f"s_cmp_eq_u32 s{S_KK}, 0")
+            e.salu(f"s_cselect_b32 s{S_T0}, s{S_MORE}, 0")
+            e.salu(f"s_cmp_eq_u32 s{S_T0}, 0")
+            e.salu("s_cbranch_scc1 L_noprefetch")
+            e.salu(f"s_add_u32 s{S_IT}, s{S_Q}, s{S_G}")
+            fetch_planes(PFR, S_IT, False)
+            e.label("L_noprefetch")
+
+        if FLAGS:
+            e.drain(vm=False)
+        if BM and not (ABL & 8) and not FLAGS:
+            e.salu(f"s_cmp_eq_u32 s{S_KK}, 0")
+            e.salu(f"s_cselect_b32 s{S_T0}, s{S_MORE}, 0")
+            e.salu(f"s_cmp_eq_u32 s{S_T0}, 0")
+            e.salu("s_cbranch_scc1 L_noprefetch")
+            e.salu(f"s_add_u32 s{S_IT}, s{S_Q}, s{S_G}")
+            fetch_planes(PFR, S_IT, False)
+            e.label("L_noprefetch")
+        mark(1)
+        e.salu(f"s_mul_i32 s{S_SS}, s{S_KK}, 3")
+        e.salu(f"s_add_u32 s{S_SS}, s{S_SS}, 2")
+        if BM:
+            e.salu(f"s_sub_u32 s{S_T0}, s{S_K}, 1")
+            e.salu(f"s_cmp_eq_u32 s{S_KK}, s{S_T0}")
+            e.salu("s_cbranch_scc1 L_rows_now")
+            e.salu(f"s_bitcmp1_b32 s{S_ACCP}, 1")
+            e.salu("s_cbranch_scc1 L_rows_held")
+            e.label("L_rows_now")
+            load_rows_now(0)
+            e.label("L_rows_held")
+            sweep_x_b(0, 1, True, None, None)
+            if FLAGS:
+                e.raw("s_waitcnt vmcnt(0)")
+                e.salu(f"s_cmp_eq_u32 s{S_HASNEXT}, 0")
+                e.salu("s_cbranch_scc1 L_noready")
+                flag_add(0, True)
+                e.label("L_noready")
+                if not (ABL & 8):
+                    prefetch_block()
+            mark(2)
+            e.salu(f"s_sub_u32 s{S_SS}, s{S_SS}, 1")
+            sweep_y_b(1, 2, (AX, TX, S_DTS[2], S_FIRSTX, S_TLX, 1, "x2"))
+            if FLAGS:
+                flag_add(1, False)
+            mark(3)
+            e.salu(f"s_sub_u32 s{S_SS}, s{S_SS}, 1")
+            sweep_x_b(2, None, False, (AY, TY, S_DTS[1], S_FIRSTY, S_TLY, 1, "y"), (AX, TX, S_DTS[0], S_FIRSTX, S_TLX, 0, "x0"))
+            mark(4)
+        else:
+            sweep_x(0, S_DTS[2])
+            mark(2)
+            e.salu(f"s_sub_u32 s{S_SS}, s{S_SS}, 1")
+            sweep_y(1, S_DTS[1])
+            mark(3)
+            e.salu(f"s_sub_u32 s{S_SS}, s{S_SS}, 1")
+            sweep_x(2, S_DTS[0])
+            mark(4)
         e.drain(vm=False)
-    if BM and not (ABL & 8) and not FLAGS:
-        e.salu(f"s_cmp_eq_u32 s{S_KK}, 0")
-        e.salu(f"s_cselect_b32 s{S_T0}, s{S_MORE}, 0")
-        e.salu(f"s_cmp_eq_u32 s{S_T0}, 0")
-        e.salu("s_cbranch_scc1 L_noprefetch")
-        e.salu(f"s_add_u32 s{S_IT}, s{S_Q}, s{S_G}")
-        fetch_planes(PFR, S_IT, False)
-        e.label("L_noprefetch")
-    mark(1)
-    e.salu(f"s_mul_i32 s{S_SS}, s{S_KK}, 3")
-    e.salu(f"s_add_u32 s{S_SS}, s{S_SS}, 2")
-    if BM:
-        e.salu(f"s_sub_u32 s{S_T0}, s{S_K}, 1")
-        e.salu(f"s_cmp_eq_u32 s{S_KK}, s{S_T0}")
-        e.salu("s_cbranch_scc1 L_rows_now")
-        e.salu(f"s_bitcmp1_b32 s{S_ACCP}, 1")
-        e.salu("s_cbranch_scc1 L_rows_held")
-        e.label("L_rows_now")
-        load_rows_now(0)
-        e.label("L_rows_held")
-        sweep_x_b(0, 1, True, None, None)
         if FLAGS:
+            e.salu(f"s_add_u32 s{S_TSTEP}, s{S_TSTEP}, 1")
+            mark(5)
+            mark(6)
+        else:
+            e.salu(f"s_cmp_eq_u32 s{S_HASNEXT}, 0")
+            e.salu("s_cbranch_scc1 L_nodts")
+            load_dts(S_KKN)
+            e.label("L_nodts")
             e.raw("s_waitcnt vmcnt(0)")
-            e.salu(f"s_cmp_eq_u32 s{S_HASNEXT}, 0")
-            e.salu("s_cbranch_scc1 L_noready")
-            flag_add(0, True)
-            e.label("L_noready")
-            if not (ABL & 8):
-                prefetch_block()
-        mark(2)
-        e.salu(f"s_sub_u32 s{S_SS}, s{S_SS}, 1")
-        sweep_y_b(1, 2, (AX, TX, S_DTS[2], S_FIRSTX, S_TLX, 1, "x2"))
-        if FLAGS:
-            flag_add(1, False)
-        mark(3)
-        e.salu(f"s_sub_u32 s{S_SS}, s{S_SS}, 1")
-        sweep_x_b(2, None, False, (AY, TY, S_DTS[1], S_FIRSTY, S_TLY, 1, "y"), (AX, TX, S_DTS[0], S_FIRSTX, S_TLX, 0, "x0"))
-        mark(4)
-    else:
-        sweep_x(0, S_DTS[2])
-        mark(2)
-        e.salu(f"s_sub_u32 s{S_SS}, s{S_SS}, 1")
-        sweep_y(1, S_DTS[1])
-        mark(3)
-        e.salu(f"s_sub_u32 s{S_SS}, s{S_SS}, 1")
-        sweep_x(2, S_DTS[0])
-        mark(4)
-    e.drain(vm=False)
-    if FLAGS:
-        e.salu(f"s_add_u32 s{S_TSTEP}, s{S_TSTEP}, 1")
-        mark(5)
-        mark(6)
-    else:
-        e.salu(f"s_cmp_eq_u32 s{S_HASNEXT}, 0")
-        e.salu("s_cbranch_scc1 L_nodts")
-        load_dts(S_KKN)
-        e.label("L_nodts")
-        e.raw("s_waitcnt vmcnt(0)")
-        e.vm = []
-        mark(5)
-        if not (ABL & 4) and not (ABL & 1024):
-            e.raw("s_barrier")
-        e.drain(vm=False)
-        mark(6)
-    stage(5)
-    if not (ABL & 4):
-        e.salu(f"s_xor_b32 s{S_SET}, s{S_SET}, {3 * RECP_B}")
-    e.salu(f"s_sub_u32 s{S_KK}, s{S_KK}, 1")
-    e.salu(f"s_cmp_ge_i32 s{S_KK}, 0")
-    e.salu("s_cbranch_scc1 L_step")
+            e.vm = []
+            mark(5)
+            if not (ABL & 4) and not (ABL & 1024):
+                e.raw("s_barrier")
+            e.drain(vm=False)
+            mark(6)
+        stage(5)
+        if not (ABL & 4):
+            e.salu(f"s_xor_b32 s{S_SET}, s{S_SET}, {3 * RECP_B}")
+        e.salu(f"s_sub_u32 s{S_KK}, s{S_KK}, 1")
+        e.salu(f"s_cmp_ge_i32 s{S_KK}, 0")
+        e.salu("s_cbranch_scc1 L_step")
     stage(6)
     if FLAGS:
         e.raw("s_waitcnt vmcnt(0)")
@@ -1335,11 +1582,43 @@
     return "\n".join(e.out) + "\n" + desc, info
 
 
+def parse_spec(spec):
+    head, _, abl = spec.partition("a")
+    mode = {"b": "B", "c": "C"}.get(head[-1], "A")
+    return int(head.rstrip("bc")), int(abl or 0), mode
+
+
+def step_loop_counts(text):
+    lines = text.split("\n")
+    i0 = lines.index("L_step:")
+    i1 = next(i for i in range(i0, len(lines)) if lines[i].split(";")[0].split() == ["s_cbranch_scc1", "L_step"])
+    c = dict(valu=0, salu=0, lds=0, vmem=0, waitcnt=0, nop=0, swap=0)
+    for ln in lines[i0 + 1:i1 + 1]:
+        t = ln.split(";")[0].split()
+        if not t or t[0].endswith(":") or t[0].startswith("."):
+            continue
+        op = t[0]
+        if op.startswith("v_"):
+            c["valu"] += 1
+            c["swap"] += op.startswith("v_permlane32_swap")
+        elif op.startswith("ds_"):
+            c["lds"] += 1
+        elif op.startswith(("global_", "buffer_")):
+            c["vmem"] += 1
+        elif op == "s_waitcnt":
+            c["waitcnt"] += 1
+        elif op == "s_nop":
+            c["nop"] += 1
+        else:
+            assert op.startswith("s_"), op
+            c["salu"] += 1
+    c["total"] = sum(v for k, v in c.items() if k != "swap")
+    return c
+
+
 if __name__ == "__main__":
     spec = sys.argv[1]
-    head, _, abl = spec.partition("a")
-    mode = "B" if head.endswith("b") else "A"
-    text, info = gen(int(head.rstrip("b")), int(abl or 0), mode)
+    text, info = gen(*parse_spec(spec))
     with open(sys.argv[2], "w") as f:
         f.write(text)
     print(info, file=sys.stderr)
diff --git a/cnn-with-pde_amd/csrc/pde_adi_asm.hip b/cnn-with-pde_amd/csrc/pde_adi_asm.hip
--- a/cnn-with-pde_amd/csrc/pde_adi_asm.hip
+++ b/cnn-with-pde_amd/csrc/pde_adi_asm.hip
@@ -37,7 +37,7 @@
         const char* on = getenv("PDE_ASM_BWD");
         if (on && on[0] == '0') return nullptr;
         const char* want = getenv("PDE_ASM_VARIANT");
-        std::string w = want ? want : "8b";
+        std::string w = want ? want : "8c";
         for (Variant& x : g_variants)
             if (w == x.spec) return &x;
         return nullptr;
```

Result: faster. 1.167 Msamples/s (median of 6 runs) (+3.2%).
